# ersanjay16/Assignment--2-Group7-distributed-K-means

Measured on AMD Instinct MI355X. Metric: Lloyd iters/sec + points/sec, N=100M d=64 k=256, 1–8 GPUs; % of roofline, higher is better.
Workload: dtype f32; 1 GPU; c3: N=100000000 d=64 k=256; N=100000000, d=64, k=256, compute_sse=False, parallelism=dp1 (rows sharded, one RCCL all-reduce of k*(d+1) f64 per step)

## Files before the change

assignment--2-group7-distributed-k-means_amd/_lib.py:

```python
from __future__ import annotations

import ctypes
import os
import threading

HERE = os.path.dirname(os.path.abspath(__file__))
_KM_LIB = os.environ.get("KM_LIB")
LIB_PATH = os.path.join(HERE, "libkmeans_amd.so") if _KM_LIB in (None, "", "diag") else _KM_LIB
ROOT = os.path.dirname(HERE)
HEADER = os.path.join(ROOT, "include", "kmeans_amd.h")

KM_ABI_VERSION = 6
KM_OK = 0
KM_EMPTY = 1

KM_K_ASSIGN, KM_K_RESOLVE, KM_K_STATS, KM_K_UPDATE, KM_K_PREP, KM_K_SEED = range(6)
KERNEL_KINDS = {"assign": KM_K_ASSIGN, "resolve": KM_K_RESOLVE, "stats": KM_K_STATS, "update": KM_K_UPDATE,
                "prep": KM_K_PREP, "seed": KM_K_SEED}


KM_STOP_CONVERGED, KM_STOP_EMPTY, KM_STOP_NONFINITE = 1, 2, 3
KM_MAX_BATCH = 32


class KmStatus(ctypes.Structure):
    _fields_ = [("sse", ctypes.c_double), ("max_shift", ctypes.c_double), ("n_empty", ctypes.c_int32),
                ("nonfinite", ctypes.c_int32), ("q_rerank", ctypes.c_int32), ("q_full", ctypes.c_int32),
                ("ran", ctypes.c_int32), ("stop_reason", ctypes.c_int32), ("repaired", ctypes.c_int32),
                ("reserved", ctypes.c_int32)]


class KmInfo(ctypes.Structure):
    _fields_ = [("n", ctypes.c_int64), ("d", ctypes.c_int32), ("dp", ctypes.c_int32), ("k", ctypes.c_int32),
                ("kp", ctypes.c_int32), ("path", ctypes.c_int32), ("n_cu", ctypes.c_int32),
                ("device", ctypes.c_int32), ("fused_stats", ctypes.c_int32),
                ("delta_stats", ctypes.c_int32)]


_P = ctypes.c_void_p
_I32 = ctypes.c_int32
_I64 = ctypes.c_int64
_D = ctypes.c_double
_PD = ctypes.POINTER(ctypes.c_double)
_PI32 = ctypes.POINTER(ctypes.c_int32)
_PI64 = ctypes.POINTER(ctypes.c_int64)
_PF = ctypes.POINTER(ctypes.c_float)

SIGNATURES = {
    "km_abi_version": [],
    "km_device_count": [ctypes.POINTER(ctypes.c_int)],
    "km_create": [ctypes.c_int, ctypes.POINTER(_P)],
    "km_destroy": [_P],
    "km_set_stream": [_P, _P],
    "km_sync": [_P],
    "km_info_get": [_P, ctypes.POINTER(KmInfo)],
    "km_gated_rows": [_P, _PI64],
    "km_stats_route": [_P, _PI32, _PI32, _PI32, _PI32, _PI32],
    "km_load_begin": [_P, _I64, _I32],
    "km_load_rows": [_P, _I64, _PF, _I64],
    "km_generate_blobs": [_P, _I64, _I32, _I64, _I32, ctypes.c_float, ctypes.c_float, ctypes.c_uint64],
    "km_set_weights": [_P, _I64, _PD, _I64],
    "km_clear_weights": [_P],
    "km_sum_x": [_P, _PD],
    "km_set_sse": [_P, _I32],
    "km_set_screen": [_P, _I32],
    "km_get_screen": [_P, ctypes.POINTER(ctypes.c_int32)],
    "km_set_centroids": [_P, _PD, _I32, _I32],
    "km_get_centroids": [_P, _I32, _PD],
    "km_assign_stats": [_P],
    "km_stats_buffer": [_P, ctypes.POINTER(_P), _PI64],
    "km_bind_stats_buffer": [_P, _P],
    "km_update": [_P, ctypes.POINTER(KmStatus), _PI64],
    "km_batch_begin": [_P],
    "km_update_async": [_P, _D, _I64],
    "km_set_layout": [_P, _PI64, _I32, _I64, _I32],
    "km_repair_state": [_P, _PI32, _PI32],
    "km_repair_buffer": [_P, ctypes.POINTER(_P), _PI64],
    "km_bind_repair_buffer": [_P, _P],
    "km_repair_apply_async": [_P],
    "km_batch_end": [_P, ctypes.POINTER(KmStatus), _PI64, _PI32],
    "km_replace_rows": [_P, _PI32, _PD, _I32],
    "km_commit": [_P],
    "km_gather_rows": [_P, _PI64, _I32, _PD],
    "km_bernoulli_sample": [_P, ctypes.POINTER(ctypes.c_uint64), _PI64, _PI64, _I32, ctypes.c_double, _PI64,
                            ctypes.c_int64, _PI64],
    "km_seed_begin": [_P],
    "km_seed_update": [_P, _I32, _PD],
    "km_seed_sample": [_P, ctypes.c_uint64, _I32, _I64, _D, _D, _PI64, _I64, _PI64],
    "km_seed_weights": [_P, _I32, _PI64],
    "km_seed_read": [_P, _PD, _PI32],
    "km_seed_end": [_P],
    "km_predict": [_P, _PI32],
    "km_labels": [_P, _PI32],
    "km_profile": [_P, _I32],
    "km_profile_every": [_P, _I32],
    "km_prof_read": [_P, _I32, _PD, _PI64],
}

_lock = threading.Lock()
_lib = None


class KmError(RuntimeError):
    pass


def _pin_runtime():
    try:
        import torch
    except Exception:
        pass


def load(path: str = None):
    global _lib
    path = path or LIB_PATH
    with _lock:
        if _lib is not None:
            return _lib
        if not os.path.exists(path):
            raise KmError(f"HIP extension not built: {path} is missing "
                          f"(run `python -c 'import __graft_entry__ as g; g.build()'` or "
                          f"`make -C {os.path.join(HERE, 'csrc')}`)")
        _pin_runtime()
        lib = ctypes.CDLL(path, mode=ctypes.RTLD_GLOBAL)
        for name, args in SIGNATURES.items():
            fn = getattr(lib, name)
            fn.argtypes = args
            fn.restype = ctypes.c_int
        lib.km_last_error.argtypes = []
        lib.km_last_error.restype = ctypes.c_char_p
        _lib = lib
        return lib


def check(rc: int, what: str = "") -> int:
    if rc < 0:
        msg = load().km_last_error().decode(errors="replace")
        raise KmError(f"{what or 'kmeans_amd'} failed ({rc}): {msg}")
    return rc


def device_count() -> int:
    lib = load()
    n = ctypes.c_int(0)
    check(lib.km_device_count(ctypes.byref(n)), "km_device_count")
    return n.value


def exported_symbols():
    return list(SIGNATURES) + ["km_last_error"]
```

assignment--2-group7-distributed-k-means_amd/csrc/km_internal.h:

```cpp
#pragma once
#include <hip/hip_ext.h>
#include <hip/hip_runtime.h>
#include <stdint.h>

#include "../../include/kmeans_amd.h"

namespace km {

struct LaunchTiming {
  hipEvent_t start = nullptr, stop = nullptr;
};
extern thread_local LaunchTiming g_timing;
#define KM_TIMED_LAUNCH(KERNEL, GRID, BLOCK, LDS, STREAM, ...)                                               \
  do {                                                                                                     \
    if (::km::g_timing.start) {                                                                            \
      hipExtLaunchKernelGGL(KERNEL, GRID, BLOCK, LDS, STREAM, ::km::g_timing.start, ::km::g_timing.stop, 0, \
                            __VA_ARGS__);                                                                  \
      ::km::g_timing = ::km::LaunchTiming{};                                                               \
    } else {                                                                                               \
      hipLaunchKernelGGL(KERNEL, GRID, BLOCK, LDS, STREAM, __VA_ARGS__);                                    \
    }                                                                                                      \
  } while (0)

struct QEntry {
  uint32_t row;
  uint32_t i1;
  uint32_t i2;
  uint32_t kind;
};

struct DevStatus {
  double sse;
  double max_shift;
  int32_t n_empty;
  int32_t nonfinite;
  int32_t q_rerank;
  int32_t q_full;
  int32_t ran;
  int32_t stop;
  int32_t repaired;
  int32_t pad;
};
static_assert(sizeof(DevStatus) == 48, "layout of km_status");


struct QLayout {
  uint32_t seg;
  uint32_t nwaves;
};

struct Geometry {
  int64_t n;
  int32_t d;
  int32_t dp;
  int32_t k;
  int32_t kp;
};

hipError_t launch_prep_centroids(const double* C64, const Geometry& g, float* C32, double* cn2, float* cmax,
                                 float* cabs, double* C64T, double* C64P, const int* gate, hipStream_t s);
hipError_t launch_prep_small(const double* C64, const Geometry& g, float* C32, float* cmax, const int* gate,
                             hipStream_t s);
hipError_t launch_prep_split(const float* C32, const Geometry& g, const double* cn2, const float* xabs,
                             const float* cabs, _Float16* Chi, _Float16* Clo, float* cn2s, const int* gate, hipStream_t s);
hipError_t launch_absmax(const float* X, int64_t nfloats, float* out, hipStream_t s);
struct SmallTail {
  uint32_t* queue;
  uint32_t* qctr;
  uint32_t* done;
  int fold;
  const double* old;
  double* out;
  int64_t* counts;
  DevStatus* st;
  int* gate;
  double stop_tol;
  int dev_repair;
  float* C32n;
  float* cmaxn;
  int kp;
  uint32_t* qout = nullptr;
  int rev = 0;
};
hipError_t launch_assign_small(const float* X, const Geometry& g, const float* C32, const double* C64,
                               const float* cmax, int32_t* labels, double* stats, int fuse_stats, int want_sse,
                               int n_cu, const int* gate, hipStream_t s, const SmallTail& tail);
bool small_path_ok(const Geometry& g);
hipError_t launch_assign_mfma(const float* X, const Geometry& g, const _Float16* Chi, const _Float16* Clo,
                              const float* cn2s, const float* cmax, const float* xabs, const float* cabs,
                              int32_t* labels, QEntry* queue, uint32_t* qcount, int n_cu, QLayout* ql,
                              const int* gate, hipStream_t s, uint32_t* cand = nullptr, uint32_t* cand_ctr = nullptr,
                              uint32_t cand_cap = 0, int one = 0,
                              const float* C32 = nullptr, uint2* chg = nullptr, uint32_t* chg_cnt = nullptr);
int cand_rec_words();
size_t queue_capacity(int64_t n, int n_cu);
size_t qcount_words(int n_cu);
bool mfma_path_ok(const Geometry& g);
hipError_t launch_resolve(const float* X, const Geometry& g, const double* C64, const double* C64T,
                          const QEntry* queue, const uint32_t* qcount, const QLayout& ql, int32_t* labels,
                          double* stats, int n_cu, const int* gate, hipStream_t s, double* sse = nullptr,
                          const uint32_t* cand = nullptr, uint32_t cand_cap = 0, int delta = 0,
                          const float* sse_c32 = nullptr, uint2* chg = nullptr, const uint32_t* chg_cnt = nullptr,
                          const float* C32 = nullptr, const float* cmax = nullptr);
bool fused_path_ok(const Geometry& g);
#ifdef KM_DIAG
#endif
int diag_env(const char* name, int dflt);
enum { KM_SCREEN_X3 = 0, KM_SCREEN_X3_REFINE = 1, KM_SCREEN_FAST1 = 2, KM_SCREEN_FAST2 = 3 };
bool fast_path_ok(const Geometry& g);
hipError_t launch_fused(const float* X, const float* xnorm, const Geometry& g, const _Float16* Chi,
                        const _Float16* Clo, uint4* ChiF, uint4* CloF, const float* cn2s, const float* bnd,
                        const float* xabs, const float* cabs, int32_t* labels, QEntry* queue, uint32_t* qcount,
                        double* stats, int with_stats, int mode, int n_cu, QLayout* ql, const int* gate,
                        hipStream_t s, const float* C32, const float* cmax, float* bal, const double* C64P,
                        double* sse);
hipError_t launch_bound_consts(const float* cmax, const float* xabs, const float* cabs, const Geometry& g, float* bnd,
                               const int* gate, hipStream_t s);
bool fused16_ok(const Geometry& g);
hipError_t launch_row_norm(const float* X, const Geometry& g, float* xnorm, hipStream_t s);
bool stats_needs_sort(const Geometry& g, int extra);
void stats_ranges(const Geometry& g, int* fr_out, int* kr_out, int extra);
size_t sorted_stats_words(int64_t n, int k);
hipError_t launch_stats(const float* X, const Geometry& g, const int32_t* labels, const double* w, double* stats,
                        int n_cu, const int* gate, hipStream_t s, const double* C64, int c64s, const float* C32);
hipError_t launch_stats_sorted(const float* X, const Geometry& g, const int32_t* labels, const double* w,
                               double* stats, uint32_t* scratch, const double* C64P, int n_cu, const int* gate,
                               hipStream_t s);
bool update_one_ok(const Geometry& g);
hipError_t launch_update(double* stats, const double* C64_old, const Geometry& g, double* C64_new,
                         double* work, int64_t* counts, const uint32_t* qcount, uint32_t nq, DevStatus* status,
                         int* gate, double stop_tol, int dev_repair, hipStream_t s, int clear = 0,
                         float* C32 = nullptr, float* cmax = nullptr, int corr = 0, const double* wdiv = nullptr);
hipError_t launch_sum_x(const float* X, const Geometry& g, double* out, hipStream_t s);
hipError_t launch_scatter_rows(const int64_t* ids, const double* rows, int32_t n, int d, double* C, hipStream_t s);
hipError_t launch_gather_rows(const float* X, const Geometry& g, const int64_t* idx, int32_t n, double* out,
                              hipStream_t s);
hipError_t launch_repair(int* gate, const int64_t* counts, const Geometry& g, int64_t total, double neg_log_delta,
                         uint64_t seed, int32_t* empty, int32_t* pcounts, int64_t* picks, int64_t* samples, int cp,
                         const int64_t* sizes, const int64_t* bases, int nparts, const float* X, int64_t row0,
                         const double* C_old, double* C_new, DevStatus* st, double tol, hipStream_t s);
hipError_t launch_repair_pick(int* gate, const int64_t* counts, const Geometry& g, int64_t total,
                              double neg_log_delta, uint64_t seed, int32_t* empty, int32_t* pcounts, int64_t* picks,
                              int64_t* samples, int cp, const int64_t* sizes, const int64_t* bases, int nparts,
                              const float* X, int64_t row0, DevStatus* st, double* rows, int32_t* pending,
                              hipStream_t s);
hipError_t launch_repair_apply(int* gate, const Geometry& g, const int32_t* empty, const double* C_old,
                               double* C_new, DevStatus* st, double tol, const double* rows, const int32_t* pending,
                               hipStream_t s);
hipError_t launch_bernoulli(const uint64_t* seeds, const int64_t* sizes, const int64_t* bases, int nparts,
                            double fraction, int64_t* out, int cp, int32_t* counts, hipStream_t s);
bool s1_ok(const Geometry& g);
size_t s1_table_entries(const Geometry& g);
hipError_t launch_s1_color(const float* C32, const Geometry& g, int32_t* perm, const int* gate, hipStream_t s);
hipError_t launch_s1_prep(const double* C64, const float* C32, const Geometry& g, const int32_t* perm,
                          const float* cmax, const float* xabs, const float* cabs, float* cft, float* cn2o,
                          uint4* img, float* cst, const int* gate, hipStream_t s);
struct S1GateBufs;
hipError_t launch_s1(const float* X, const float* xnorm, const Geometry& g, const uint4* img, const float* cn2o,
                     const float* cft, const int32_t* perm, const float* cst, int32_t* labels,
                     QEntry* queue, uint32_t* qcount, uint2* chg, uint32_t* chg_cnt, int delta, int n_cu,
                     QLayout* ql, const int* gate, hipStream_t s, int rev = 0, double* sse = nullptr,
                     const S1GateBufs* gt = nullptr, int gdense = 0);
struct S1GateBufs {
  float* marg;
  uint2* wl;
  uint32_t* wl_cnt;
  double* cref;
  double* acc;
  float* accud;
};
bool s1_gate_ok(const Geometry& g);
hipError_t launch_s1_gate(const Geometry& g, const double* C64, const int32_t* labels, const S1GateBufs& b, int init,
                          const int32_t* init_dev, int n_cu, const int* gate, hipStream_t s);
size_t s1_chg_entries(const Geometry& g, int n_cu);
size_t s1_wave_slots(int n_cu);
bool s1_delta_ok(const Geometry& g, int n_cu);
hipError_t launch_s1_delta(const float* X, const Geometry& g, const uint2* chg, const uint32_t* chg_cnt,
                           double* stats, int n_cu, const int* gate, hipStream_t s, const uint32_t* qcount = nullptr);
hipError_t launch_chg_delta(const float* X, const Geometry& g, const uint2* chg, const uint32_t* chg_cnt, int nw,
                            uint32_t seg, double* stats, int n_cu, const int* gate, hipStream_t s,
                            const uint32_t* qcount = nullptr);
hipError_t launch_s1_apply(double* stats, double* full, int64_t len, int mode, const int* gate, hipStream_t s);
hipError_t launch_gen_blobs(float* X, const Geometry& g, int64_t row_offset, int32_t n_centers, float box,
                            float stddev, uint64_t seed, hipStream_t s);

__host__ __device__ inline uint64_t splitmix64(uint64_t z) {
  z += 0x9E3779B97F4A7C15ull;
  z = (z ^ (z >> 30)) * 0xBF58476D1CE4E5B9ull;
  z = (z ^ (z >> 27)) * 0x94D049BB133111EBull;
  return z ^ (z >> 31);
}

hipError_t launch_seed_init(double* D2, int32_t* near, int64_t n, hipStream_t s);
int seed_fold_blocks(int64_t n, int n_cu);
int seed_sample_blocks(int64_t n, int n_cu);
hipError_t launch_seed_fold(const float* X, const Geometry& g, const double* C64, const int32_t* labels,
                            int32_t first_id, double* D2, int32_t* near, double* part, int n_cu, hipStream_t s);
hipError_t launch_seed_sample(const double* D2, int64_t n, uint64_t seed, int32_t round, int64_t row0, double ell,
                              double phi, uint32_t* cnt, int64_t* offs, int64_t* out, int64_t cap, int n_cu,
                              hipStream_t s);
hipError_t launch_seed_weights(const int32_t* near, int64_t n, int32_t m_total, unsigned long long* counts, int n_cu,
                               hipStream_t s);

}
```

assignment--2-group7-distributed-k-means_amd/csrc/km_runtime.hip:

```cpp
#include <stdlib.h>
#include <string.h>

#include <algorithm>
#include <cmath>
#include <string>
#include <utility>
#include <vector>

#include "../../include/kmeans_amd.h"
#include "km_internal.h"

namespace {
thread_local std::string g_err;

int fail(int code, const std::string& msg) {
  g_err = msg;
  return code;
}

#define KM_HIP(call)                                                                               \
  do {                                                                                             \
    hipError_t e_ = (call);                                                                        \
    if (e_ != hipSuccess)                                                                          \
      return fail(KM_ERR_HIP, std::string(#call) + ": " + hipGetErrorString(e_) + " (" +           \
                                  std::to_string((int)e_) + ")");                                  \
  } while (0)

#define KM_REQUIRE(cond, code, msg) \
  do {                              \
    if (!(cond)) return fail(code, msg); \
  } while (0)

template <class T>
void dfree(T*& p) {
  if (p) (void)hipFree(p);
  p = nullptr;
}
template <class T>
void hfree(T*& p) {
  if (p) (void)hipHostFree(p);
  p = nullptr;
}

constexpr int kAllowedDp[] = {16, 32, 48, 64, 96, 128, 192, 256};

bool fused_disabled() { return km::diag_env("KM_FUSED", 1) == 0; }

size_t stats_len(const km::Geometry& g) { return (size_t)g.k * (g.d + 1) + 1; }
size_t stats_cap(const km::Geometry& g) { return stats_len(g) + (size_t)g.k; }

int choose_dp(int d) {
  for (int v : kAllowedDp)
    if (d <= v) return v;
  return (d + 15) / 16 * 16;
}
}

struct km_ctx {
  int device = 0;
  int n_cu = 256;
  hipStream_t own_stream = nullptr;
  hipStream_t stream = nullptr;
  km::Geometry g{};
  bool loaded = false;
  bool have_c = false;
  int path = 0;
  bool fused = false;
  int screen = km::KM_SCREEN_X3_REFINE;
  bool fast_blocked = false;
  int screen_forced = -1;
  bool s1 = false;
  bool mdelta_geo = false;
  uint2* chg_m = nullptr;
  uint32_t* chg_m_cnt = nullptr;
  bool s1_recolor = true;
  int s1_color_age = 0;
  int s1_batches = 0;
  int32_t* s1_perm = nullptr;
  float* s1_cft = nullptr;
  float* s1_cn2o = nullptr;
  uint4* s1_img = nullptr;
  float* s1_cst = nullptr;
  double* stats_full = nullptr;
  uint2* chg = nullptr;
  uint32_t* chg_cnt = nullptr;
  bool delta_ready = false;
  km::S1GateBufs gt{nullptr, nullptr, nullptr, nullptr, nullptr, nullptr};
  bool bounds_valid = false;
  bool last_gated = false;
  uint32_t gated_nw = 0;
  bool gated_dense = false;
  const int32_t* gate_init_dev = nullptr;
  bool x3_stale = true;
  bool sweep_rev = false;
  int stats_pending = 0;
  bool last_delta = false;
  bool sse_corr = false;
  float* bal = nullptr;
  bool stats_clean = false;
  bool rep_armed = false;
  float* X = nullptr;
  double* w = nullptr;
  int32_t* labels = nullptr;
  km::QEntry* queue = nullptr;
  uint32_t* qcount = nullptr;
  uint32_t* small_ctr = nullptr;
  bool assign_pending = false;
  bool stats_exported = false;
  uint32_t* cand = nullptr;
  uint32_t* cand_ctr = nullptr;
  uint32_t cand_cap = 0;
  km::QLayout ql{0, 0};
  double* moments = nullptr;
  bool want_sse = false;
  int64_t* idx_scratch = nullptr;
  double* rows_scratch = nullptr;
  int64_t scratch_rows = 0;
  int k_alloc = 0;
  double* C64_cur = nullptr;
  double* C64_new = nullptr;
  double* C64T = nullptr;
  double* C64P = nullptr;
  float* C32 = nullptr;
  _Float16* Chi = nullptr;
  _Float16* Clo = nullptr;
  double* cn2 = nullptr;
  float* cn2s = nullptr;
  float* cmax = nullptr;
  float* cabs = nullptr;
  float* xabs = nullptr;
  float* xnorm = nullptr;
  uint4* ChiF = nullptr;
  uint4* CloF = nullptr;
  float* bnd = nullptr;
  uint32_t* sort_scratch = nullptr;
  size_t sort_words = 0;
  double* stats_own = nullptr;
  double* stats = nullptr;
  double* work = nullptr;
  int64_t* counts_dev = nullptr;
  km::DevStatus* status_dev = nullptr;
  km::DevStatus* status_host = nullptr;
  int64_t* counts_host = nullptr;
  int* gate = nullptr;
  km::DevStatus* hist = nullptr;
  km::DevStatus* hist_host = nullptr;
  int64_t* hist_counts = nullptr;
  int64_t* hist_counts_host = nullptr;
  bool in_batch = false;
  int batch_n = 0;
  double* slot_cur[KM_MAX_BATCH] = {};
  double* slot_new[KM_MAX_BATCH] = {};
  bool rep_enabled = false;
  int rep_nparts = 0;
  int64_t rep_total = 0, rep_row0 = 0, rep_maxpart = 0;
  int64_t* rep_sizes = nullptr;
  int64_t* rep_bases = nullptr;
  int rep_cp = 0, rep_k = 0;
  int32_t* rep_empty = nullptr;
  int32_t* rep_pcounts = nullptr;
  int64_t* rep_picks = nullptr;
  int64_t* rep_samples = nullptr;
  int rep_mode = 0;
  double* rep_rows = nullptr;
  double* rep_rows_own = nullptr;
  int32_t* rep_pending = nullptr;
  bool rep_wait = false;
  double rep_tol = 0.0;
  bool rep_fold = false;
  bool seed_on = false;
  double* seed_d2 = nullptr;
  int32_t* seed_near = nullptr;
  double* seed_part = nullptr;
  uint32_t* seed_cnt = nullptr;
  int64_t* seed_offs = nullptr;
  int64_t* seed_out = nullptr;
  int64_t seed_out_cap = 0;
  float* pinned = nullptr;
  size_t pinned_floats = 0;
  hipEvent_t staged[2] = {nullptr, nullptr};
  int prof = 0;
  int prof_period = 1;
  int64_t prof_tick[KM_K_COUNT] = {};
  const double* prep_of = nullptr;
  struct Timed {
    hipEvent_t first, second;
    int64_t batch;
    int slot;
  };
  std::vector<Timed> ev[KM_K_COUNT];
  int64_t batch_seq = 0;
  std::vector<hipEvent_t> pool;

  hipEvent_t take_event() {
    if (!pool.empty()) {
      hipEvent_t e = pool.back();
      pool.pop_back();
      return e;
    }
    hipEvent_t e = nullptr;
    (void)hipEventCreate(&e);
    return e;
  }
};

namespace {

size_t stats_len(const km_ctx* c) { return c->w ? stats_cap(c->g) : stats_len(c->g); }

struct ProfScope {
  km_ctx* c;
  int kind;
  bool in_dispatch;
  hipEvent_t a = nullptr, b = nullptr;
  bool on;
  ProfScope(km_ctx* ctx, int k, bool dispatch = false)
      : c(ctx), kind(k), in_dispatch(dispatch),
        on(((c->prof >> k) & 1) && (c->prof_tick[k]++ % c->prof_period) == 0) {
    if (on) {
      a = c->take_event();
      b = c->take_event();
      if (in_dispatch)
        km::g_timing = km::LaunchTiming{a, b};
      else
        (void)hipEventRecord(a, c->stream);
    }
  }
  ~ProfScope() {
    if (on) {
      if (!in_dispatch) {
        (void)hipEventRecord(b, c->stream);
      } else if (km::g_timing.start) {
        km::g_timing = km::LaunchTiming{};
        (void)hipEventRecord(a, c->stream);
        (void)hipEventRecord(b, c->stream);
      }
      c->ev[kind].push_back({a, b, c->in_batch ? c->batch_seq : -1, c->batch_n});
    }
  }
};

void free_centroids(km_ctx* c) {
  dfree(c->C64_cur);
  dfree(c->C64_new);
  dfree(c->C64T);
  dfree(c->C64P);
  dfree(c->C32);
  dfree(c->Chi);
  dfree(c->Clo);
  dfree(c->cn2);
  dfree(c->cn2s);
  dfree(c->ChiF);
  dfree(c->CloF);
  dfree(c->bnd);
  c->bal = nullptr;
  dfree(c->cmax);
  dfree(c->cabs);
  dfree(c->stats_own);
  dfree(c->s1_perm);
  dfree(c->s1_cft);
  dfree(c->s1_cn2o);
  dfree(c->s1_img);
  dfree(c->s1_cst);
  dfree(c->stats_full);
  dfree(c->chg);
  dfree(c->chg_cnt);
  dfree(c->gt.marg);
  dfree(c->gt.wl);
  dfree(c->gt.wl_cnt);
  dfree(c->gt.cref);
  dfree(c->gt.acc);
  dfree(c->gt.accud);
  c->bounds_valid = false;
  c->last_gated = false;
  c->s1 = false;
  c->mdelta_geo = false;
  c->delta_ready = false;
  c->stats_pending = 0;
  dfree(c->work);
  dfree(c->counts_dev);
  dfree(c->status_dev);
  hfree(c->status_host);
  hfree(c->counts_host);
  dfree(c->hist);
  hfree(c->hist_host);
  dfree(c->hist_counts);
  hfree(c->hist_counts_host);
  c->in_batch = false;
  c->batch_n = 0;
  if (c->stats != nullptr && c->stats != c->stats_own) {
  }
  c->stats = nullptr;
  c->k_alloc = 0;
  c->have_c = false;
}

void free_seed(km_ctx* c) {
  dfree(c->seed_d2);
  dfree(c->seed_near);
  dfree(c->seed_part);
  dfree(c->seed_cnt);
  dfree(c->seed_offs);
  dfree(c->seed_out);
  c->seed_out_cap = 0;
  c->seed_on = false;
}

void free_data(km_ctx* c) {
  free_seed(c);
  dfree(c->X);
  dfree(c->w);
  dfree(c->labels);
  dfree(c->queue);
  dfree(c->qcount);
  dfree(c->small_ctr);
  c->assign_pending = false;
  dfree(c->cand);
  dfree(c->cand_ctr);
  c->cand_cap = 0;
  dfree(c->chg_m);
  dfree(c->chg_m_cnt);
  dfree(c->moments);
  dfree(c->xabs);
  dfree(c->xnorm);
  dfree(c->sort_scratch);
  c->sort_words = 0;
  dfree(c->idx_scratch);
  dfree(c->rows_scratch);
  c->scratch_rows = 0;
  c->loaded = false;
  c->delta_ready = false;
}

int ensure_x3(km_ctx* c) {
  if (!c->x3_stale) return KM_OK;
  KM_HIP(km::launch_prep_split(c->C32, c->g, c->cn2, c->xabs, c->cabs, c->Chi, c->Clo, c->cn2s, c->gate, c->stream));
  KM_HIP(km::launch_bound_consts(c->cmax, c->xabs, c->cabs, c->g, c->bnd, c->gate, c->stream));
  c->x3_stale = false;
  return KM_OK;
}

int prep(km_ctx* c, const double* src) {
  ProfScope ps(c, KM_K_PREP);
  c->prep_of = src;
  if (c->path == 1) {
    KM_HIP(km::launch_prep_small(src, c->g, c->C32, c->cmax, c->gate, c->stream));
    return KM_OK;
  }
  KM_HIP(km::launch_prep_centroids(src, c->g, c->C32, c->cn2, c->cmax, c->cabs, c->C64T, c->C64P, c->gate,
                                   c->stream));
  c->x3_stale = true;
  if (!c->s1) {
    const int rc = ensure_x3(c);
    if (rc != KM_OK) return rc;
  }
  if (c->s1) {
    if (c->s1_recolor) {
      KM_HIP(km::launch_s1_color(c->C32, c->g, c->s1_perm, c->gate, c->stream));
      c->s1_recolor = false;
    }
    KM_HIP(km::launch_s1_prep(src, c->C32, c->g, c->s1_perm, c->cmax, c->xabs, c->cabs, c->s1_cft, c->s1_cn2o,
                              c->s1_img, c->s1_cst, c->gate, c->stream));
  }
  return KM_OK;
}

int ensure_scratch(km_ctx* c, int64_t rows) {
  if (rows <= c->scratch_rows) return KM_OK;
  dfree(c->idx_scratch);
  dfree(c->rows_scratch);
  KM_HIP(hipMalloc(&c->idx_scratch, sizeof(int64_t) * rows));
  KM_HIP(hipMalloc(&c->rows_scratch, sizeof(double) * rows * std::max(1, c->g.d)));
  c->scratch_rows = rows;
  return KM_OK;
}

int prep(km_ctx* c) { return prep(c, c->C64_cur); }

void free_repair(km_ctx* c) {
  dfree(c->rep_empty);
  dfree(c->rep_pcounts);
  dfree(c->rep_picks);
  dfree(c->rep_samples);
  dfree(c->rep_rows_own);
  dfree(c->rep_pending);
  c->rep_rows = nullptr;
  c->rep_cp = 0;
  c->rep_k = 0;
}

void drop_layout(km_ctx* c) {
  free_repair(c);
  dfree(c->rep_sizes);
  dfree(c->rep_bases);
  c->rep_enabled = false;
  c->rep_armed = false;
  c->rep_wait = false;
  c->rep_mode = 0;
  c->rep_nparts = 0;
  c->rep_total = 0;
  c->rep_maxpart = 0;
  c->rep_row0 = 0;
}

double sample_fraction(int64_t num, int64_t total) {
  const double fraction = (double)num / (double)total;
  const double gamma = -std::log(0.00005) / (double)total;
  return std::min(1.0, fraction + gamma + std::sqrt(gamma * gamma + 2.0 * gamma * fraction));
}

int ensure_repair(km_ctx* c) {
  if (c->rep_k == c->g.k && c->rep_pcounts) return KM_OK;
  free_repair(c);
  const double f = sample_fraction(std::min<int64_t>(c->g.k, std::max<int64_t>(c->rep_total - 1, 1)),
                                   std::max<int64_t>(c->rep_total, 1));
  const double cpd = 4.0 * f * (double)c->rep_maxpart + 64.0;
  KM_REQUIRE(cpd < (double)(1 << 26), KM_ERR_ARG, "km_update_async: repair buffers too large");
  c->rep_cp = (int)cpd;
  const size_t slots = (size_t)c->rep_cp * c->rep_nparts;
  KM_HIP(hipMalloc(&c->rep_empty, sizeof(int32_t) * c->g.k));
  KM_HIP(hipMalloc(&c->rep_pcounts, sizeof(int32_t) * c->rep_nparts));
  KM_HIP(hipMemsetAsync(c->rep_pcounts, 0, sizeof(int32_t) * c->rep_nparts, c->stream));
  KM_HIP(hipMalloc(&c->rep_picks, sizeof(int64_t) * slots));
  KM_HIP(hipMalloc(&c->rep_samples, sizeof(int64_t) * slots));
  KM_HIP(hipMalloc(&c->rep_pending, sizeof(int32_t)));
  KM_HIP(hipMemsetAsync(c->rep_pending, 0, sizeof(int32_t), c->stream));
  if (c->rep_mode == 2) {
    KM_HIP(hipMalloc(&c->rep_rows_own, sizeof(double) * (size_t)c->g.k * std::max(1, c->g.d)));
    c->rep_rows = c->rep_rows_own;
  }
  c->rep_k = c->g.k;
  return KM_OK;
}

bool next_sweep(km_ctx* c) {
  if ((double)c->g.n * c->g.dp * 4.0 > 8.0 * (1ull << 30)) return false;
  c->sweep_rev = !c->sweep_rev;
  return c->sweep_rev;
}

km::SmallTail small_tail(km_ctx* c) {
  km::SmallTail t{};
  t.queue = reinterpret_cast<uint32_t*>(c->queue);
  t.qctr = c->small_ctr;
  t.done = c->small_ctr + 1;
  t.kp = c->g.kp;
  t.qout = c->qcount;
  t.rev = next_sweep(c);
  return t;
}

bool fold_ok(km_ctx* c) {
  return c->in_batch && c->path == 1 && km::update_one_ok(c->g) && c->stats == c->stats_own && !c->stats_exported &&
         !(c->rep_enabled && c->rep_armed) && !c->w;
}

int run_assign(km_ctx* c, bool with_stats);

#ifndef KM_PAIR_RESCORE
#define KM_PAIR_RESCORE 1
#endif

bool one_screen(km_ctx* c) {
  if (c->path != 2 || c->fused || c->g.dp % 32 != 0 || c->g.dp > 256) return false;
  if (c->screen_forced == KM_SCREEN_ONE) return true;
  return c->screen_forced < 0 && !c->s1;
}

bool use_s1(km_ctx* c, bool with_stats) {
  if (!c->s1) return false;
  if (c->screen_forced >= 0 && c->screen_forced != KM_SCREEN_S1) return false;
  return !with_stats || (c->delta_ready && !c->stats_exported && km::s1_delta_ok(c->g, c->n_cu));
}

int stats_route(const km_ctx* c) {
  if (c->w) return km::stats_needs_sort(c->g, 2) ? 2 : 1;
  if (c->path == 1 || c->fused) return 0;
  return km::stats_needs_sort(c->g, 1) ? 2 : 1;
}

int run_stats(km_ctx* c, bool sse) {
  const km::Geometry& g = c->g;
  ProfScope ps(c, KM_K_STATS);
  if (stats_route(c) == 2) {
    const size_t words = km::sorted_stats_words(g.n, g.k);
    if (words > c->sort_words) {
      dfree(c->sort_scratch);
      KM_HIP(hipMalloc(&c->sort_scratch, sizeof(uint32_t) * words));
      c->sort_words = words;
    }
    KM_REQUIRE(!c->w || c->path == 2, KM_ERR_UNSUPPORTED,
               "km_assign_stats: weighted statistics need the MFMA path at this k");
    KM_HIP(km::launch_stats_sorted(c->X, g, c->labels, c->w, c->stats, c->sort_scratch, sse ? c->C64P : nullptr,
                                   c->n_cu, c->gate, c->stream));
  } else {
    const bool small = c->path == 1;
    KM_HIP(km::launch_stats(c->X, g, c->labels, c->w, c->stats, c->n_cu, c->gate, c->stream,
                            sse ? (small ? c->C64_cur : c->C64P) : nullptr, small ? g.d : g.dp,
                            sse ? c->C32 : nullptr));
  }
  return KM_OK;
}

int apply_stats(km_ctx* c, const double** upd_src = nullptr, bool clear = false) {
  const int kind = c->stats_pending;
  c->stats_pending = 0;
  if (upd_src) *upd_src = c->stats;
  if (!c->s1 && !c->mdelta_geo) return KM_OK;
  const bool keep = kind == 2 || kind == 1;
  const bool zero = kind == 2 && clear && upd_src;
  if (keep)
    KM_HIP(km::launch_s1_apply(c->stats, c->stats_full, (int64_t)stats_len(c), kind == 2 ? (zero ? 2 : 1) : 0,
                               c->gate, c->stream));
  if (zero) {
    *upd_src = c->stats_full;
    c->stats_clean = true;
  }
  c->delta_ready = keep;
  return KM_OK;
}

int take_sse_corr(km_ctx* c) {
  const bool v = c->sse_corr;
  c->sse_corr = false;
  return v ? 1 : 0;
}

int flush_assign(km_ctx* c) {
  if (!c->assign_pending) return KM_OK;
  c->assign_pending = false;
  return run_assign(c, true);
}

int run_assign(km_ctx* c, bool with_stats) {
  const km::Geometry& g = c->g;
  if (c->prep_of != c->C64_cur) {
    const int rc = prep(c);
    if (rc != KM_OK) return rc;
  }
  c->ql = km::QLayout{0, 0};
  if (with_stats && c->stats_pending == 2) {
    c->delta_ready = false;
  }
  const bool sse = with_stats && c->want_sse;
  double* sse_slot = c->stats + (size_t)g.k * (g.d + 1);
  const bool bounds_were_valid = c->bounds_valid;
  c->bounds_valid = false;
  if (!use_s1(c, with_stats)) c->gate_init_dev = nullptr;
  if (with_stats) c->last_gated = false;
  if (with_stats && !c->stats_clean) KM_HIP(hipMemsetAsync(c->stats, 0, sizeof(double) * stats_len(c), c->stream));
  if (with_stats) c->stats_clean = false;
  if (c->path == 1) {
    ProfScope ps(c, KM_K_ASSIGN, true);
    KM_HIP(km::launch_assign_small(c->X, g, c->C32, c->C64_cur, c->cmax, c->labels, c->stats, with_stats ? 1 : 0,
                                   sse ? 1 : 0, c->n_cu, c->gate, c->stream, small_tail(c)));
    c->ql = km::QLayout{0, g.n > 0 ? 1u : 0u};
    return KM_OK;
  }
  if (with_stats) {
    c->stats_pending = 1;
    c->last_delta = false;
    c->sse_corr = false;
  }
  if (use_s1(c, with_stats)) {
    double* s1_sse = sse ? sse_slot : nullptr;
    const bool gated = with_stats && !s1_sse && c->fused && g.n > 0 && km::s1_gate_ok(g);
    bool gdense = false;
    if (gated) {
      if (!c->gt.marg) {
        KM_HIP(hipMalloc(&c->gt.marg, sizeof(float) * (size_t)g.n));
        KM_HIP(hipMalloc(&c->gt.wl, sizeof(uint2) * km::s1_chg_entries(g, c->n_cu)));
        KM_HIP(hipMalloc(&c->gt.wl_cnt, sizeof(uint32_t) * km::s1_wave_slots(c->n_cu)));
        KM_HIP(hipMalloc(&c->gt.cref, sizeof(double) * (size_t)g.k * g.d));
        KM_HIP(hipMemsetAsync(c->gt.cref, 0, sizeof(double) * (size_t)g.k * g.d, c->stream));
        KM_HIP(hipMalloc(&c->gt.acc, sizeof(double) * (size_t)g.k));
        KM_HIP(hipMalloc(&c->gt.accud, sizeof(float) * 2 * (size_t)g.k));
        KM_HIP(hipMemsetAsync(c->gt.acc, 0, sizeof(double) * (size_t)g.k, c->stream));
        KM_HIP(hipMemsetAsync(c->gt.accud, 0, sizeof(float) * 2 * (size_t)g.k, c->stream));
      }
      gdense = !bounds_were_valid;
      ProfScope ps(c, KM_K_PREP);
      KM_HIP(km::launch_s1_gate(g, c->C64_cur, c->labels, c->gt, gdense ? 2 : 0, c->gate_init_dev, c->n_cu, c->gate,
                                c->stream));
    }
    c->gate_init_dev = nullptr;
    {
      ProfScope ps(c, KM_K_ASSIGN, true);
      KM_HIP(km::launch_s1(c->X, c->xnorm, g, c->s1_img, c->s1_cn2o, c->s1_cft, c->s1_perm, c->s1_cst,
                           c->labels, c->queue, c->qcount, c->chg, c->chg_cnt, with_stats ? 1 : 0, c->n_cu,
                           &c->ql, c->gate, c->stream, gated ? 0 : next_sweep(c), s1_sse,
                           gated ? &c->gt : nullptr, gdense ? 1 : 0));
    }
    if (gated) {
      c->bounds_valid = true;
      c->last_gated = true;
      c->gated_nw = c->ql.nwaves;
      c->gated_dense = gdense;
    }
    {
      ProfScope ps(c, KM_K_RESOLVE);
      KM_HIP(km::launch_resolve(c->X, g, c->C64_cur, c->C64T, c->queue, c->qcount, c->ql, c->labels, nullptr,
                                c->n_cu, c->gate, c->stream, s1_sse, nullptr, 0, with_stats ? 1 : 0,
                                s1_sse ? c->C32 : nullptr, c->chg, c->chg_cnt, c->C32, c->cmax));
    }
    if (with_stats) {
      ProfScope ps(c, KM_K_STATS);
      KM_HIP(km::launch_s1_delta(c->X, g, c->chg, c->chg_cnt, c->stats, c->n_cu, c->gate, c->stream, c->qcount));
    }
    if (with_stats) {
      c->stats_pending = 2;
      c->last_delta = true;
      c->sse_corr = s1_sse != nullptr;
    }
    return KM_OK;
  }
  if (c->fused) {
    {
      const int rc = ensure_x3(c);
      if (rc != KM_OK) return rc;
    }
    {
      ProfScope ps(c, KM_K_ASSIGN, true);
      KM_HIP(km::launch_fused(c->X, c->xnorm, g, c->Chi, c->Clo, c->ChiF, c->CloF, c->cn2s, c->bnd, c->xabs, c->cabs,
                              c->labels, c->queue, c->qcount, c->stats, with_stats ? 1 : 0,
                              (with_stats || c->screen >= km::KM_SCREEN_FAST1) ? c->screen : km::KM_SCREEN_X3_REFINE,
                              c->n_cu, &c->ql, c->gate, c->stream, c->C32, c->cmax, c->bal, c->C64P,
                              sse ? sse_slot : nullptr));
    }
    {
      ProfScope ps(c, KM_K_RESOLVE);
      KM_HIP(km::launch_resolve(c->X, g, c->C64_cur, c->C64T, c->queue, c->qcount, c->ql, c->labels,
                                with_stats ? c->stats : nullptr, c->n_cu, c->gate, c->stream,
                                sse ? sse_slot : nullptr, nullptr, 0, 0, nullptr, nullptr, nullptr, c->C32, c->cmax));
    }
    return KM_OK;
  }
  if (c->s1 && !c->fused && (c->screen_forced < 0 || c->screen_forced == KM_SCREEN_S1)) {
    {
      ProfScope ps(c, KM_K_ASSIGN, true);
      KM_HIP(km::launch_s1(c->X, c->xnorm, g, c->s1_img, c->s1_cn2o, c->s1_cft, c->s1_perm, c->s1_cst, c->labels,
                           c->queue, c->qcount, c->chg, c->chg_cnt, 0, c->n_cu, &c->ql, c->gate, c->stream,
                           next_sweep(c)));
    }
    {
      ProfScope ps(c, KM_K_RESOLVE);
      KM_HIP(km::launch_resolve(c->X, g, c->C64_cur, c->C64T, c->queue, c->qcount, c->ql, c->labels, nullptr,
                                c->n_cu, c->gate, c->stream, nullptr, nullptr, 0, 0, nullptr, nullptr, nullptr, c->C32,
                                c->cmax));
    }
  } else {
  if (!c->cand && g.dp <= 256) {
    const int64_t cap = std::min<int64_t>(std::max<int64_t>(g.n, 1024), (int64_t)1 << 22);
    KM_HIP(hipMalloc(&c->cand, sizeof(uint32_t) * km::cand_rec_words() * (size_t)cap));
    KM_HIP(hipMalloc(&c->cand_ctr, sizeof(uint32_t)));
    c->cand_cap = (uint32_t)cap;
  }
  {
    const int rc = ensure_x3(c);
    if (rc != KM_OK) return rc;
  }
  const bool mdelta = with_stats && c->mdelta_geo && c->delta_ready && !c->want_sse && !c->stats_exported;
  if (mdelta && !c->chg_m) {
    KM_HIP(hipMalloc(&c->chg_m, sizeof(uint2) * km::queue_capacity(std::max<int64_t>(g.n, 1), c->n_cu)));
    KM_HIP(hipMalloc(&c->chg_m_cnt, sizeof(uint32_t) * km::qcount_words(c->n_cu)));
  }
  {
    ProfScope ps(c, KM_K_ASSIGN);
    KM_HIP(km::launch_assign_mfma(c->X, g, c->Chi, c->Clo, c->cn2s, c->cmax, c->xabs, c->cabs, c->labels, c->queue,
                                  c->qcount, c->n_cu, &c->ql, c->gate, c->stream, c->cand, c->cand_ctr,
                                  c->cand_cap, one_screen(c) ? 1 : 0, KM_PAIR_RESCORE ? c->C32 : nullptr,
                                  mdelta ? c->chg_m : nullptr, mdelta ? c->chg_m_cnt : nullptr));
  }
  {
    ProfScope ps(c, KM_K_RESOLVE);
    KM_HIP(km::launch_resolve(c->X, g, c->C64_cur, c->C64T, c->queue, c->qcount, c->ql, c->labels, nullptr, c->n_cu,
                              c->gate, c->stream, nullptr, c->cand, c->cand_cap, mdelta ? 1 : 0, nullptr,
                              mdelta ? c->chg_m : nullptr, mdelta ? c->chg_m_cnt : nullptr, c->C32, c->cmax));
  }
  if (mdelta) {
    ProfScope ps(c, KM_K_STATS);
    KM_HIP(km::launch_chg_delta(c->X, g, c->chg_m, c->chg_m_cnt, (int)c->ql.nwaves, c->ql.seg, c->stats, c->n_cu,
                                c->gate, c->stream, c->qcount));
    c->stats_pending = 2;
    c->last_delta = true;
    return KM_OK;
  }
  }
  if (with_stats) return run_stats(c, sse);
  return KM_OK;
}

int run_assign_weighted(km_ctx* c) {
  int rc = run_assign(c, false);
  if (rc != KM_OK) return rc;
  c->delta_ready = false;
  c->stats_pending = 0;
  c->last_delta = false;
  c->last_gated = false;
  c->sse_corr = false;
  c->gate_init_dev = nullptr;
  KM_HIP(hipMemsetAsync(c->stats, 0, sizeof(double) * stats_len(c), c->stream));
  c->stats_clean = false;
  return run_stats(c, c->want_sse);
}

const double* wdiv_of(const km_ctx* c, const double* src) { return c->w ? src + stats_len(c->g) : nullptr; }

}

extern "C" {

int km_abi_version(void) { return KM_ABI_VERSION; }

const char* km_last_error(void) { return g_err.c_str(); }

int km_device_count(int* out) {
  KM_REQUIRE(out, KM_ERR_ARG, "km_device_count: null out");
  int n = 0;
  hipError_t e = hipGetDeviceCount(&n);
  if (e != hipSuccess) n = 0;
  *out = n;
  return KM_OK;
}

int km_create(int device, km_ctx** out) {
  KM_REQUIRE(out, KM_ERR_ARG, "km_create: null out");
  *out = nullptr;
  int n = 0;
  KM_HIP(hipGetDeviceCount(&n));
  KM_REQUIRE(device >= 0 && device < n, KM_ERR_ARG,
             "km_create: device " + std::to_string(device) + " out of range (" + std::to_string(n) + " devices)");
  KM_HIP(hipSetDevice(device));
  hipDeviceProp_t prop;
  KM_HIP(hipGetDeviceProperties(&prop, device));
  KM_REQUIRE(std::string(prop.gcnArchName).rfind("gfx950", 0) == 0, KM_ERR_UNSUPPORTED,
             std::string("km_create: kernels are built for gfx950 (MI355X), device is ") + prop.gcnArchName);
  km_ctx* c = new km_ctx();
  c->device = device;
  c->n_cu = prop.multiProcessorCount;
  hipError_t e = hipStreamCreateWithFlags(&c->own_stream, hipStreamNonBlocking);
  if (e != hipSuccess) {
    delete c;
    return fail(KM_ERR_HIP, std::string("hipStreamCreate: ") + hipGetErrorString(e));
  }
  c->stream = c->own_stream;
  e = hipMalloc(&c->gate, sizeof(int));
  if (e == hipSuccess) e = hipMemset(c->gate, 0, sizeof(int));
  if (e != hipSuccess) {
    (void)hipStreamDestroy(c->own_stream);
    delete c;
    return fail(KM_ERR_HIP, std::string("km_create: ") + hipGetErrorString(e));
  }
  *out = c;
  return KM_OK;
}

int km_destroy(km_ctx* c) {
  if (!c) return KM_OK;
  (void)hipSetDevice(c->device);
  (void)hipStreamSynchronize(c->stream);
  free_centroids(c);
  free_data(c);
  hfree(c->pinned);
  for (auto& e : c->staged)
    if (e) (void)hipEventDestroy(e);
  for (auto& v : c->ev)
    for (auto& p : v) {
      (void)hipEventDestroy(p.first);
      (void)hipEventDestroy(p.second);
    }
  for (auto e : c->pool) (void)hipEventDestroy(e);
  dfree(c->gate);
  free_repair(c);
  dfree(c->rep_sizes);
  dfree(c->rep_bases);
  if (c->own_stream) (void)hipStreamDestroy(c->own_stream);
  delete c;
  return KM_OK;
}

int km_set_stream(km_ctx* c, void* s) {
  KM_REQUIRE(c, KM_ERR_ARG, "null ctx");
  KM_HIP(hipSetDevice(c->device));
  {
    const int rcf = flush_assign(c);
    if (rcf != KM_OK) return rcf;
  }
  KM_HIP(hipStreamSynchronize(c->stream));
  c->stream = s ? reinterpret_cast<hipStream_t>(s) : c->own_stream;
  return KM_OK;
}

int km_sync(km_ctx* c) {
  KM_REQUIRE(c, KM_ERR_ARG, "null ctx");
  KM_HIP(hipSetDevice(c->device));
  {
    const int rcf = flush_assign(c);
    if (rcf != KM_OK) return rcf;
  }
  KM_HIP(hipStreamSynchronize(c->stream));
  return KM_OK;
}

int km_info_get(km_ctx* c, km_info* out) {
  KM_REQUIRE(c && out, KM_ERR_ARG, "null arg");
  out->n = c->g.n;
  out->d = c->g.d;
  out->dp = c->g.dp;
  out->k = c->g.k;
  out->kp = c->g.kp;
  out->path = c->path;
  out->n_cu = c->n_cu;
  out->device = c->device;
  out->fused_stats = (c->path == 1) || c->fused;
  out->delta_stats = c->last_delta ? 1 : 0;
  return KM_OK;
}

int km_gated_rows(km_ctx* c, int64_t* out) {
  KM_REQUIRE(c && out, KM_ERR_ARG, "null arg");
  *out = -1;
  if (!c->last_gated || !c->gt.wl_cnt || c->gated_nw == 0) return KM_OK;
  if (c->gated_dense) {
    *out = c->g.n;
    return KM_OK;
  }
  KM_HIP(hipSetDevice(c->device));
  std::vector<uint32_t> cnt(c->gated_nw);
  KM_HIP(hipMemcpyAsync(cnt.data(), c->gt.wl_cnt, sizeof(uint32_t) * cnt.size(), hipMemcpyDeviceToHost, c->stream));
  KM_HIP(hipStreamSynchronize(c->stream));
  int64_t total = 0;
  for (uint32_t v : cnt) total += v;
  *out = total;
  return KM_OK;
}

int km_stats_route(km_ctx* c, int32_t* route, int32_t* cluster_ranges, int32_t* kr, int32_t* feature_ranges,
                   int32_t* fr) {
  KM_REQUIRE(c && route && cluster_ranges && kr && feature_ranges && fr, KM_ERR_ARG, "km_stats_route: null arg");
  KM_REQUIRE(c->have_c && c->path != 0, KM_ERR_STATE, "km_stats_route: set centroids of a supported geometry first");
  *route = stats_route(c);
  *cluster_ranges = *kr = *feature_ranges = *fr = 0;
  if (*route == 0) return KM_OK;
  int f = 0, r = 0;
  km::stats_ranges(c->g, &f, &r, c->w ? 2 : 1);
  KM_REQUIRE(f > 0 && r > 0, KM_ERR_UNSUPPORTED, "km_stats_route: no table split for this geometry");
  *fr = f;
  *kr = r;
  *feature_ranges = c->g.dp / f;
  *cluster_ranges = (c->g.k + r - 1) / r;
  return KM_OK;
}

int km_load_begin(km_ctx* c, int64_t n, int32_t d) {
  KM_REQUIRE(c, KM_ERR_ARG, "null ctx");
  KM_REQUIRE(n >= 0 && n < (int64_t)UINT32_MAX, KM_ERR_ARG, "km_load_begin: n out of range");
  KM_REQUIRE(d > 0, KM_ERR_ARG, "km_load_begin: d must be positive");
  KM_HIP(hipSetDevice(c->device));
  {
    const int rcf = flush_assign(c);
    if (rcf != KM_OK) return rcf;
  }
  KM_HIP(hipStreamSynchronize(c->stream));
  free_data(c);
  free_centroids(c);
  drop_layout(c);
  c->g = km::Geometry{};
  c->g.n = n;
  c->g.d = d;
  c->g.dp = choose_dp(d);
  const int64_t rows = std::max<int64_t>(n, 1);
  KM_HIP(hipMalloc(&c->X, sizeof(float) * rows * c->g.dp));
  KM_HIP(hipMemsetAsync(c->X, 0, sizeof(float) * rows * c->g.dp, c->stream));
  KM_HIP(hipMalloc(&c->labels, sizeof(int32_t) * rows));
  KM_HIP(hipMalloc(&c->queue, sizeof(km::QEntry) * km::queue_capacity(rows, c->n_cu)));
  KM_HIP(hipMalloc(&c->qcount, sizeof(uint32_t) * km::qcount_words(c->n_cu)));
  KM_HIP(hipMalloc(&c->small_ctr, sizeof(uint32_t) * 3));
  KM_HIP(hipMemsetAsync(c->small_ctr, 0, sizeof(uint32_t) * 3, c->stream));
  KM_HIP(hipMalloc(&c->moments, sizeof(double) * (d + 1)));
  KM_HIP(hipMalloc(&c->xabs, sizeof(float)));
  KM_HIP(hipMalloc(&c->xnorm, sizeof(float) * rows));
  KM_HIP(hipMemsetAsync(c->xabs, 0, sizeof(float), c->stream));
  KM_HIP(hipStreamSynchronize(c->stream));
  c->loaded = true;
  return KM_OK;
}

int km_load_rows(km_ctx* c, int64_t row0, const float* rows, int64_t nrows) {
  KM_REQUIRE(c && c->loaded, KM_ERR_STATE, "km_load_rows: call km_load_begin first");
  KM_REQUIRE(row0 >= 0 && nrows >= 0 && row0 + nrows <= c->g.n, KM_ERR_ARG, "km_load_rows: rows out of range");
  if (nrows == 0) return KM_OK;
  KM_REQUIRE(rows, KM_ERR_ARG, "km_load_rows: null rows");
  KM_HIP(hipSetDevice(c->device));
  {
    const int rcf = flush_assign(c);
    if (rcf != KM_OK) return rcf;
  }
  c->delta_ready = false;
  c->bounds_valid = false;
  const int d = c->g.d, dp = c->g.dp;
  const size_t chunk_floats = (size_t)16 << 20;
  if (!c->pinned) {
    KM_HIP(hipHostMalloc(&c->pinned, 2 * chunk_floats * sizeof(float), hipHostMallocDefault));
    c->pinned_floats = chunk_floats;
    for (auto& e : c->staged) KM_HIP(hipEventCreateWithFlags(&e, hipEventDisableTiming));
  }
  const int64_t per = std::max<int64_t>(1, (int64_t)(c->pinned_floats / d));
  KM_REQUIRE((size_t)d <= c->pinned_floats, KM_ERR_ARG, "km_load_rows: row wider than the staging buffer");
  int half = 0;
  bool used[2] = {false, false};
  for (int64_t r = 0; r < nrows; r += per, half ^= 1) {
    const int64_t m = std::min(per, nrows - r);
    float* buf = c->pinned + (size_t)half * c->pinned_floats;
    if (used[half]) KM_HIP(hipEventSynchronize(c->staged[half]));
    memcpy(buf, rows + r * d, sizeof(float) * m * d);
    KM_HIP(hipMemcpy2DAsync(c->X + (row0 + r) * dp, sizeof(float) * dp, buf, sizeof(float) * d,
                            sizeof(float) * d, m, hipMemcpyHostToDevice, c->stream));
    KM_HIP(hipEventRecord(c->staged[half], c->stream));
    used[half] = true;
    KM_HIP(km::launch_absmax(c->X + (row0 + r) * dp, m * dp, c->xabs, c->stream));
    km::Geometry sub = c->g;
    sub.n = m;
    KM_HIP(km::launch_row_norm(c->X + (row0 + r) * dp, sub, c->xnorm + row0 + r, c->stream));
  }
  KM_HIP(hipStreamSynchronize(c->stream));
  return KM_OK;
}

static int weights_mode_changed(km_ctx* c) {
  c->delta_ready = false;
  c->bounds_valid = false;
  c->last_gated = false;
  c->last_delta = false;
  c->stats_pending = 0;
  c->sse_corr = false;
  c->stats_clean = false;
  c->stats = c->stats_own;
  return KM_OK;
}

int km_set_weights(km_ctx* c, int64_t row0, const double* w, int64_t nrows) {
  KM_REQUIRE(c && c->loaded, KM_ERR_STATE, "km_set_weights: call km_load_begin first");
  KM_REQUIRE(!c->in_batch, KM_ERR_STATE, "km_set_weights: inside a batch");
  KM_REQUIRE(row0 >= 0 && nrows >= 0 && row0 + nrows <= c->g.n, KM_ERR_ARG, "km_set_weights: rows out of range");
  KM_REQUIRE(nrows == 0 || w, KM_ERR_ARG, "km_set_weights: null weights");
  KM_HIP(hipSetDevice(c->device));
  {
    const int rcf = flush_assign(c);
    if (rcf != KM_OK) return rcf;
  }
  KM_HIP(hipStreamSynchronize(c->stream));
  if (!c->w) {
    const int64_t rows = std::max<int64_t>(c->g.n, 1);
    std::vector<double> ones((size_t)std::min<int64_t>(rows, (int64_t)1 << 20), 1.0);
    KM_HIP(hipMalloc(&c->w, sizeof(double) * rows));
    for (int64_t r = 0; r < rows; r += (int64_t)ones.size())
      KM_HIP(hipMemcpy(c->w + r, ones.data(), sizeof(double) * std::min<int64_t>((int64_t)ones.size(), rows - r),
                       hipMemcpyHostToDevice));
    weights_mode_changed(c);
  }
  const int64_t per = (int64_t)8 << 20;
  for (int64_t r = 0; r < nrows; r += per) {
    const int64_t m = std::min(per, nrows - r);
    KM_HIP(hipMemcpyAsync(c->w + row0 + r, w + r, sizeof(double) * m, hipMemcpyHostToDevice, c->stream));
    KM_HIP(hipStreamSynchronize(c->stream));
  }
  c->delta_ready = false;
  return KM_OK;
}

int km_clear_weights(km_ctx* c) {
  KM_REQUIRE(c, KM_ERR_ARG, "null ctx");
  KM_REQUIRE(!c->in_batch, KM_ERR_STATE, "km_clear_weights: inside a batch");
  if (!c->w) return KM_OK;
  KM_HIP(hipSetDevice(c->device));
  KM_HIP(hipStreamSynchronize(c->stream));
  dfree(c->w);
  return weights_mode_changed(c);
}

int km_generate_blobs(km_ctx* c, int64_t n, int32_t d, int64_t global_row0, int32_t n_centers, float box,
                      float stddev, uint64_t seed) {
  KM_REQUIRE(c, KM_ERR_ARG, "null ctx");
  KM_REQUIRE(n_centers > 0, KM_ERR_ARG, "n_centers must be positive");
  int rc = km_load_begin(c, n, d);
  if (rc != KM_OK) return rc;
  KM_HIP(km::launch_gen_blobs(c->X, c->g, global_row0, n_centers, box, stddev, seed, c->stream));
  KM_HIP(km::launch_absmax(c->X, c->g.n * c->g.dp, c->xabs, c->stream));
  KM_HIP(km::launch_row_norm(c->X, c->g, c->xnorm, c->stream));
  KM_HIP(hipStreamSynchronize(c->stream));
  return KM_OK;
}

int km_sum_x(km_ctx* c, double* out) {
  KM_REQUIRE(c && c->loaded && out, KM_ERR_STATE, "km_sum_x: no data");
  KM_HIP(hipSetDevice(c->device));
  KM_HIP(hipMemsetAsync(c->moments, 0, sizeof(double) * (c->g.d + 1), c->stream));
  KM_HIP(km::launch_sum_x(c->X, c->g, c->moments, c->stream));
  KM_HIP(hipMemcpyAsync(out, c->moments, sizeof(double) * c->g.d, hipMemcpyDeviceToHost, c->stream));
  KM_HIP(hipStreamSynchronize(c->stream));
  return KM_OK;
}

int km_set_screen(km_ctx* c, int32_t mode) {
  KM_REQUIRE(c, KM_ERR_ARG, "null ctx");
  KM_REQUIRE(mode >= -1 && mode <= KM_SCREEN_ONE, KM_ERR_ARG, "km_set_screen: mode must be -1..5");
#ifndef KM_DIAG
  KM_REQUIRE(mode <= km::KM_SCREEN_X3_REFINE || mode == KM_SCREEN_S1 || mode == KM_SCREEN_ONE, KM_ERR_UNSUPPORTED,
             "km_set_screen: fast screens (modes 2, 3) are in the diagnostic build only");
#endif
  c->screen_forced = mode;
  if (mode >= 0 && mode != KM_SCREEN_S1 && mode != KM_SCREEN_ONE) c->screen = mode;
  return KM_OK;
}

int km_get_screen(km_ctx* c, int32_t* mode) {
  KM_REQUIRE(c && mode, KM_ERR_ARG, "null ctx");
  *mode = (use_s1(c, true) || (c->s1 && !c->fused && (c->screen_forced < 0 || c->screen_forced == KM_SCREEN_S1)))
              ? KM_SCREEN_S1
              : one_screen(c) ? KM_SCREEN_ONE : c->screen;
  return KM_OK;
}

int km_set_sse(km_ctx* c, int32_t enable) {
  KM_REQUIRE(c, KM_ERR_ARG, "null ctx");
  {
    const int rcf = flush_assign(c);
    if (rcf != KM_OK) return rcf;
  }
  c->want_sse = enable != 0;
  return KM_OK;
}

int km_set_centroids(km_ctx* c, const double* C, int32_t k, int32_t d) {
  KM_REQUIRE(c && c->loaded, KM_ERR_STATE, "km_set_centroids: load data first");
  KM_REQUIRE(C, KM_ERR_ARG, "km_set_centroids: null C");
  KM_REQUIRE(k > 0, KM_ERR_ARG, "km_set_centroids: k must be positive");
  KM_REQUIRE(d == c->g.d, KM_ERR_ARG,
             "km_set_centroids: d=" + std::to_string(d) + " != data d=" + std::to_string(c->g.d));
  KM_HIP(hipSetDevice(c->device));
  {
    const int rcf = flush_assign(c);
    if (rcf != KM_OK) return rcf;
  }
  if (k != c->k_alloc) {
    KM_HIP(hipStreamSynchronize(c->stream));
    double* external = (c->stats && c->stats != c->stats_own) ? c->stats : nullptr;
    (void)external;
    free_centroids(c);
    c->g.k = k;
    c->g.kp = (k + 63) / 64 * 64;
    const int kp = c->g.kp, dp = c->g.dp;
    KM_HIP(hipMalloc(&c->C64_cur, sizeof(double) * k * d));
    KM_HIP(hipMalloc(&c->C64_new, sizeof(double) * k * d));
    KM_HIP(hipMalloc(&c->C64T, sizeof(double) * k * d));
    KM_HIP(hipMalloc(&c->C64P, sizeof(double) * kp * dp));
    KM_HIP(hipMalloc(&c->C32, sizeof(float) * kp * dp));
    KM_HIP(hipMalloc(&c->Chi, sizeof(_Float16) * kp * dp));
    KM_HIP(hipMalloc(&c->Clo, sizeof(_Float16) * kp * dp));
    KM_HIP(hipMalloc(&c->cn2, sizeof(double) * kp));
    KM_HIP(hipMalloc(&c->cn2s, sizeof(float) * kp));
    KM_HIP(hipMalloc(&c->ChiF, sizeof(_Float16) * kp * dp));
    KM_HIP(hipMalloc(&c->CloF, sizeof(_Float16) * kp * dp));
    KM_HIP(hipMalloc(&c->bnd, sizeof(float) * 16));
    c->bal = c->bnd + 4;
    KM_HIP(hipMalloc(&c->cmax, sizeof(float)));
    KM_HIP(hipMalloc(&c->cabs, sizeof(float)));
    KM_HIP(hipMalloc(&c->stats_own, sizeof(double) * stats_cap(c->g)));
    KM_HIP(hipMalloc(&c->work, sizeof(double) * 3 * k));
    KM_HIP(hipMalloc(&c->counts_dev, sizeof(int64_t) * k));
    KM_HIP(hipMalloc(&c->status_dev, sizeof(km::DevStatus)));
    KM_HIP(hipHostMalloc(&c->status_host, sizeof(km::DevStatus), hipHostMallocDefault));
    KM_HIP(hipHostMalloc(&c->counts_host, sizeof(int64_t) * k, hipHostMallocDefault));
    KM_HIP(hipMalloc(&c->hist, sizeof(km::DevStatus) * KM_MAX_BATCH));
    KM_HIP(hipHostMalloc(&c->hist_host, sizeof(km::DevStatus) * KM_MAX_BATCH, hipHostMallocDefault));
    KM_HIP(hipMalloc(&c->hist_counts, sizeof(int64_t) * (size_t)k * KM_MAX_BATCH));
    KM_HIP(hipHostMalloc(&c->hist_counts_host, sizeof(int64_t) * (size_t)k * KM_MAX_BATCH, hipHostMallocDefault));
    c->stats = c->stats_own;
    c->stats_clean = false;
    c->k_alloc = k;
    if (km::small_path_ok(c->g))
      c->path = 1;
    else if (km::mfma_path_ok(c->g))
      c->path = 2;
    else
      c->path = 0;
    c->fused = (c->path == 2) && km::fused_path_ok(c->g) && !fused_disabled();
    c->s1 = (c->path == 2) && (!c->fused || km::fused16_ok(c->g)) && km::s1_ok(c->g) &&
            km::diag_env("KM_S1", 1) != 0;
    c->mdelta_geo = (c->path == 2) && !c->fused && !c->s1 && c->g.dp % 32 == 0 && c->g.dp <= 128 &&
                    c->g.k <= 65535 && km::diag_env("KM_MDELTA", 1) != 0;
    if (c->mdelta_geo) KM_HIP(hipMalloc(&c->stats_full, sizeof(double) * stats_cap(c->g)));
    if (c->s1) {
      const size_t nt = km::s1_table_entries(c->g);
      KM_HIP(hipMalloc(&c->s1_perm, sizeof(int32_t) * nt));
      KM_HIP(hipMalloc(&c->s1_cft, sizeof(float) * nt * (dp + 4)));
      KM_HIP(hipMalloc(&c->s1_cn2o, sizeof(float) * kp));
      KM_HIP(hipMalloc(&c->s1_img, sizeof(_Float16) * kp * dp));
      KM_HIP(hipMalloc(&c->s1_cst, sizeof(float) * 8));
      KM_HIP(hipMalloc(&c->stats_full, sizeof(double) * stats_cap(c->g)));
      KM_HIP(hipMalloc(&c->chg, sizeof(uint2) * km::s1_chg_entries(c->g, c->n_cu)));
      KM_HIP(hipMalloc(&c->chg_cnt, sizeof(uint32_t) * km::s1_wave_slots(c->n_cu)));
    }
  }
  c->s1_recolor = true;
  c->s1_color_age = 0;
  c->s1_batches = 0;
  c->delta_ready = false;
  c->bounds_valid = false;
  c->stats_pending = 0;
  KM_HIP(hipMemcpyAsync(c->C64_cur, C, sizeof(double) * k * d, hipMemcpyHostToDevice, c->stream));
  int rc = prep(c);
  if (rc != KM_OK) return rc;
  KM_HIP(hipStreamSynchronize(c->stream));
  c->have_c = true;
  c->screen = c->screen_forced >= 0 ? c->screen_forced : km::KM_SCREEN_X3_REFINE;
  c->fast_blocked = false;
  c->rep_armed = c->rep_enabled;
  return KM_OK;
}

int km_get_centroids(km_ctx* c, int32_t which, double* out) {
  KM_REQUIRE(c && c->have_c && out, KM_ERR_STATE, "km_get_centroids: no centroids");
  KM_HIP(hipSetDevice(c->device));
  {
    const int rcf = flush_assign(c);
    if (rcf != KM_OK) return rcf;
  }
  const double* src = which ? c->C64_new : c->C64_cur;
  KM_HIP(hipMemcpyAsync(out, src, sizeof(double) * c->g.k * c->g.d, hipMemcpyDeviceToHost, c->stream));
  KM_HIP(hipStreamSynchronize(c->stream));
  return KM_OK;
// ... 651 lines not shown
```

assignment--2-group7-distributed-k-means_amd/csrc/km_s1_gate.h:

```cpp
#pragma once
#include <math.h>
#include <stdint.h>

#if defined(__HIPCC__) || defined(__CUDACC__)
#define KM_S1G_FN __host__ __device__ inline
#else
#define KM_S1G_FN inline
#endif

namespace km {

constexpr float S1G_U = 5.9604644775390625e-08f;
constexpr float S1G_TINY = 1e-30f;

KM_S1G_FN float s1g_up(float v) { return fmaf(fabsf(v), 8.0f * S1G_U, v) + S1G_TINY; }
KM_S1G_FN float s1g_dn(float v) { return fmaf(fabsf(v), -8.0f * S1G_U, v) - S1G_TINY; }

KM_S1G_FN float s1g_sqrt(float v) {
#if defined(__HIP_DEVICE_COMPILE__)
  return __builtin_amdgcn_sqrtf(v);
#else
  return sqrtf(v);
#endif
}

KM_S1G_FN float s1g_shift(double sq) {
  const double v = sqrt(sq) * (1.0 + 1e-12);
  const float f = (float)v;
  const float r = fmaf(f, 0x1p-23f, f) + S1G_TINY;
  return (r <= 3.0e38f) ? r : INFINITY;
}

KM_S1G_FN float s1g_step(float marg, float sl, float so) { return s1g_dn(marg - s1g_up(sl + so)); }

struct S1GRow {
  float is2;
  float E;
  float xlo;
  float xhi;
};

KM_S1G_FN S1GRow s1g_row(float s, float E_scaled, float xs) {
  S1GRow r;
  r.is2 = 1.0f / (s * s);
  r.E = s1g_up(E_scaled * r.is2);
  r.xhi = s1g_up(xs * (1.0f + 64.0f * S1G_U));
  r.xlo = s1g_dn(xs * (1.0f - 64.0f * S1G_U));
  return r;
}

KM_S1G_FN bool s1g_scale_ok(float s) { return s >= 0x1p-30f && s <= 0x1p30f; }

KM_S1G_FN float s1g_ub(float key, float rp, const S1GRow& r) {
  const float p = key * r.is2;
  float v = s1g_up(p + s1g_up(rp * fabsf(p)));
  v = s1g_up(v + r.E);
  v = s1g_up(v + r.xhi);
  v = !(v < 0x1p-96f) ? v : 0x1p-96f;
  return s1g_up(s1g_up(s1g_sqrt(v)));
}

KM_S1G_FN float s1g_lb(float key, float rp, const S1GRow& r) {
  const float p = key * r.is2;
  float v = s1g_dn(p - s1g_up(rp * fabsf(p)));
  v = s1g_dn(v - r.E);
  v = s1g_dn(v + r.xlo);
  return (v >= 0x1p-96f) ? s1g_dn(s1g_dn(s1g_sqrt(v))) : 0.0f;
}

KM_S1G_FN float s1g_margin(float lb, float ub) {
  const float m = s1g_dn(lb - ub);
  return (fabsf(m) <= 3.0e38f) ? m : 0.0f;
}

KM_S1G_FN double s1g_acc_add(double acc, float sl, float so) {
  return (acc + ((double)sl + (double)so)) * (1.0 + 0x1p-50);
}
KM_S1G_FN float s1g_acc_up(double acc) {
  const float f = (float)acc;
  const float r = fmaf(f, 0x1p-23f, f) + S1G_TINY;
  return (r <= 3.0e38f) ? r : INFINITY;
}
KM_S1G_FN float s1g_acc_dn(double acc) {
  if (!(acc <= 3.0e38)) return 0.0f;
  const float f = (float)acc;
  const float r = fmaf(f, -0x1p-23f, f) - S1G_TINY;
  return r > 0.0f ? r : 0.0f;
}
KM_S1G_FN double s1g_acc_pass(double acc, float sl, float so, float top, bool reset, float* up, float* dn) {
  const bool wild = !(top <= 3.0e38f);
  const double a = (reset || wild) ? 0.0 : s1g_acc_add(acc, sl, so);
  *up = (wild && !reset) ? INFINITY : s1g_acc_up(a);
  *dn = s1g_acc_dn(a);
  return a;
}
KM_S1G_FN float s1g_base(float marg, float acc_dn) {
  const float b = s1g_dn(marg + acc_dn);
  return (fabsf(b) <= 3.0e38f) ? b : 0.0f;
}
KM_S1G_FN bool s1g_keep(float base, float acc_up) { return base > acc_up; }

KM_S1G_FN float s1g_xnorm(float xs) {
  float v = s1g_up(xs * (1.0f + 64.0f * S1G_U));
  v = !(v < 0x1p-96f) ? v : 0x1p-96f;
  return s1g_up(s1g_up(s1g_sqrt(v)));
}

}
```

assignment--2-group7-distributed-k-means_amd/csrc/km_screen1.hip:

```cpp
#include <float.h>

#include <type_traits>

#include "km_internal.h"
#include "km_s1_gate.h"
#include "km_s1_ring.h"

namespace km {

namespace {

typedef _Float16 f16x8 __attribute__((ext_vector_type(8)));
typedef float f32x4 __attribute__((ext_vector_type(4)));
typedef float f32x2 __attribute__((ext_vector_type(2)));
typedef _Float16 f16x2 __attribute__((ext_vector_type(2)));

constexpr float U24 = 5.9604644775390625e-08f;
constexpr float U16 = 4.8828125e-04f;
#ifndef KM_S1_LMAX
#define KM_S1_LMAX 8
#endif
constexpr int S1_LMAX = KM_S1_LMAX;
#ifndef KM_S1_NBUF
#define KM_S1_NBUF 0
#endif
#ifndef KM_S1_ABL
#define KM_S1_ABL 0
#endif
constexpr int ceil_log2_c(int v) { return v <= 1 ? 0 : 1 + ceil_log2_c((v + 1) / 2); }
#ifndef KM_S1_W12
#define KM_S1_W12 1
#endif
#ifndef KM_S1_W12_C4
#define KM_S1_W12_C4 1
#endif
constexpr int s1_waves(int ns2, int nb) {
  return ((KM_S1_W12 && ns2 == 2 && nb == 8) || (KM_S1_W12_C4 && ns2 == 1 && nb == 32)) ? 12 : 8;
}

constexpr int S1_MAX_WAVES = 12;
constexpr int s1_ring(int ns2, int nb) { return s1_waves(ns2, nb) == 12 ? 12 : 16; }

constexpr bool s1_batched(int ns2) { return ns2 <= 2; }
#ifndef KM_S1_SERP
#define KM_S1_SERP 1
#endif
#ifndef KM_S1_TT
#define KM_S1_TT 1
#endif
constexpr int s1_tiles(int ns2) { return ns2 == 1 ? KM_S1_TT : 1; }

constexpr size_t s1_lds_bytes(int ns2, int nb, bool table) {
  const int dp = 32 * ns2, kp = 32 * nb, nt = 32 << ceil_log2_c(nb);
  return (size_t)kp * dp * 2 + (table ? (size_t)nt * (dp + 4) * 4 : 0) + (size_t)kp * 4 + (size_t)nt * 4 +
         (s1_batched(ns2) ? (size_t)s1_waves(ns2, nb) * s1_ring(ns2, nb) * (dp * 4 + 16 + 128) : 0);
}
constexpr bool s1_table_global(int ns2, int nb) { return s1_lds_bytes(ns2, nb, true) > 160 * 1024; }
#ifndef KM_S1_GATE
#define KM_S1_GATE 1
#endif
constexpr size_t s1_gate_ring_lds(int ns2, int nb) { return (size_t)s1_waves(ns2, nb) * s1_ring(ns2, nb) * 4; }
constexpr size_t s1_gate_lds(int ns2, int nb) { return s1_gate_ring_lds(ns2, nb) + (size_t)32 * nb * 4; }
constexpr bool s1_gated_with(int ns2, int nb, size_t extra) {
  return KM_S1_GATE && s1_batched(ns2) && s1_tiles(ns2) == 1 && !s1_table_global(ns2, nb) &&
         s1_lds_bytes(ns2, nb, true) + extra <= 160 * 1024;
}
constexpr bool s1_gated(int ns2, int nb) { return s1_gated_with(ns2, nb, s1_gate_lds(ns2, nb)); }
constexpr bool s1_gated_kept(int ns2, int nb) {
  return s1_gated(ns2, nb) == s1_gated_with(ns2, nb, s1_gate_ring_lds(ns2, nb));
}
static_assert(s1_gated_kept(2, 2) && s1_gated_kept(2, 4) && s1_gated_kept(2, 6) && s1_gated_kept(2, 8) &&
                  s1_gated_kept(1, 2) && s1_gated_kept(1, 4) && s1_gated_kept(1, 6) && s1_gated_kept(1, 8) &&
                  s1_gated_kept(1, 12) && s1_gated_kept(1, 16),
              "the lower totals' LDS table must not cost a geometry its gate");
static_assert(!KM_S1_GATE || !KM_S1_W12 || s1_gated(2, 8), "the c3 geometry is gated");


__device__ __forceinline__ uint32_t f2u(float v) { return __float_as_uint(v); }
__device__ __forceinline__ float u2f(uint32_t v) { return __uint_as_float(v); }

__device__ __forceinline__ float min_raw(float a, float b) {
  float r;
  asm("v_min_f32 %0, %1, %2" : "=v"(r) : "v"(a), "v"(b));
  return r;
}
__device__ __forceinline__ float min3_raw(float a, float b, float c) {
  float r;
  asm("v_min3_f32 %0, %1, %2, %3" : "=v"(r) : "v"(a), "v"(b), "v"(c));
  return r;
}

__device__ __forceinline__ float quad_min(float v) {
  auto p = __builtin_amdgcn_permlane16_swap(f2u(v), f2u(v), false, false);
  v = min_raw(u2f(p[0]), u2f(p[1]));
  p = __builtin_amdgcn_permlane32_swap(f2u(v), f2u(v), false, false);
  return min_raw(u2f(p[0]), u2f(p[1]));
}
__device__ __forceinline__ float quad_sum(float v) {
  auto p = __builtin_amdgcn_permlane16_swap(f2u(v), f2u(v), false, false);
  v = u2f(p[0]) + u2f(p[1]);
  p = __builtin_amdgcn_permlane32_swap(f2u(v), f2u(v), false, false);
  return u2f(p[0]) + u2f(p[1]);
}
__device__ __forceinline__ int32_t quad_min_i(int32_t v) {
  auto p = __builtin_amdgcn_permlane16_swap((uint32_t)v, (uint32_t)v, false, false);
  v = min((int32_t)p[0], (int32_t)p[1]);
  p = __builtin_amdgcn_permlane32_swap((uint32_t)v, (uint32_t)v, false, false);
  return min((int32_t)p[0], (int32_t)p[1]);
}
__device__ __forceinline__ int32_t mono(uint32_t b) { return (int32_t)(b ^ ((uint32_t)((int32_t)b >> 31) >> 1)); }
__device__ __forceinline__ uint32_t unmono(int32_t v) { return (uint32_t)v ^ ((uint32_t)(v >> 31) >> 1); }
__device__ __forceinline__ uint32_t quad_add_u(uint32_t v) {
  auto p = __builtin_amdgcn_permlane16_swap(v, v, false, false);
  v = p[0] + p[1];
  p = __builtin_amdgcn_permlane32_swap(v, v, false, false);
  return p[0] + p[1];
}

__device__ __forceinline__ float s1_scale(float xabs, float cabs) {
  const float m = fmaxf(xabs, cabs);
  if (!(m > 0.0f) || !(m < 3.0e38f)) return 1.0f;
  int e;
  (void)frexpf(m, &e);
  return ldexpf(1.0f, 14 - e);
}

}

struct S1Geo {
  int nb, mb, ns2;
};

template <int DPC, int NTH>
__global__ __launch_bounds__(NTH) void k_s1_color(const float* __restrict__ C32, int k, int dp, int nb, int mb,
                                                  int32_t* __restrict__ perm, const int* __restrict__ gate) {
  if (*gate) return;
  __shared__ unsigned int cmin[32];
  __shared__ int cnt[32];
  __shared__ int cls[NTH];
  const int t = threadIdx.x;
  float cv[DPC];
#pragma unroll
  for (int f = 0; f < DPC; ++f) cv[f] = (t < k && f < dp) ? C32[(size_t)t * dp + f] : 0.0f;
  if (t < 32) cnt[t] = 0;
  cls[t] = -1;
  __syncthreads();
  for (int j = 0; j < k; ++j) {
    if (t < 32) cmin[t] = 0x7F800000u;
    __syncthreads();
    if (t < j) {
      float s = 0.0f;
#pragma unroll
      for (int f = 0; f < DPC; ++f) {
        const float df = cv[f] - C32[(size_t)j * dp + f];
        s = fmaf(df, df, s);
      }
      atomicMin(&cmin[cls[t]], __float_as_uint(s));
    }
    __syncthreads();
    if (t < 64) {
      uint64_t key = 0;
      if (t < 32 && cnt[t] < nb) key = ((uint64_t)(cmin[t] + 1u) << 8) | (uint64_t)(31 - t);
#pragma unroll
      for (int o = 32; o >= 1; o >>= 1) {
        const uint64_t other = __shfl_xor(key, o);
        key = other > key ? other : key;
      }
      if (t == 0) {
        const int c = 31 - (int)(key & 255u);
        const int m = cnt[c];
        cls[j] = c;
        cnt[c] = m + 1;
        perm[(c << mb) | m] = j;
      }
    }
    __syncthreads();
  }
  for (int i = t; i < (32 << mb); i += blockDim.x) {
    const int c = i >> mb, m = i & ((1 << mb) - 1);
    if (m >= cnt[c]) perm[i] = -1;
  }
}

__global__ __launch_bounds__(64) void k_s1_prep(const double* __restrict__ C64, const float* __restrict__ C32, int k,
                                                int d, int dp, S1Geo sg, const int32_t* __restrict__ perm,
                                                const float* __restrict__ cmax, const float* __restrict__ xabs,
                                                const float* __restrict__ cabs, float* __restrict__ cft,
                                                float* __restrict__ cn2o, uint4* __restrict__ img,
                                                float* __restrict__ cst,
                                                const int* __restrict__ gate) {
  if (*gate) return;
  const int b = blockIdx.x, th = threadIdx.x;
  const int nt = 32 << sg.mb;
  const float s = s1_scale(*xabs, *cabs);
  const int cs = dp + 4;
  if (b < nt) {
    const int chain = b >> sg.mb, member = b & ((1 << sg.mb) - 1);
    const int j = member < sg.nb ? perm[b] : -1;
    for (int f = th; f < cs; f += 64) cft[(size_t)b * cs + f] = (j >= 0 && f < d) ? C32[(size_t)j * dp + f] : 0.0f;
    if (member >= sg.nb) return;
    const int cb = chain >> 4, M = chain & 15;
    if (th == 0) {
      double nn = 0.0;
      if (j >= 0)
        for (int f = 0; f < d; ++f) nn = fma(C64[(size_t)j * d + f], C64[(size_t)j * d + f], nn);
      cn2o[32 * member + 16 * cb + M] = j >= 0 ? (float)(nn * (double)s * (double)s) : 1e30f;
    }
    const int fq = dp / 4;
    if (th < 4 * sg.ns2) {
      const int q = th / sg.ns2, t = th - q * sg.ns2;
      f16x8 v;
#pragma unroll
      for (int e = 0; e < 8; ++e) {
        const int f = fq * q + 8 * t + e;
        v[e] = (j >= 0 && f < d) ? (_Float16)(-2.0f * s * C32[(size_t)j * dp + f]) : (_Float16)0.0f;
      }
      img[((size_t)(member * 2 + cb) * sg.ns2 + t) * 64 + 16 * q + M] = __builtin_bit_cast(uint4, v);
    }
    return;
  }
  if (th == 0) {
    const float cm = *cmax * s, ca = *cabs * (1.0f + U24) * s, xa = *xabs * s;
    const float sq = sqrtf((float)dp) * 1.0001f, nm = (float)sg.ns2;
    const float e1 = 1.25f * (2.0f * s * cm * (2.0f * U16 + U16 * U16 + 2.0f * U24) +
                              nm * 4.0f * U24 * 2.0f * s * cm * (1.0f + 2.0f * U16) +
                              ldexpf(1.0f, -25) * s * sq * (1.0f + U16));
    const float e0 = 1.25f * (U24 * cm * cm + nm * (4.0f * U24 * cm * cm +
                                                     28.0f * U24 * 2.0f * ca * xa * (1.0f + U16) * (1.0f + U16)) +
                              ldexpf(1.0f, -24) * sq * cm);
    cst[0] = s;
    cst[1] = e1 * 1.0001f;
    cst[2] = e0 * 1.0001f + 1e-30f;
    cst[3] = U24 * *cmax * 1.01f + 1e-37f;
  }
}

struct S1Args {
  const float* X;
  const float* xnorm;
  int64_t n;
  int k, d;
  uint32_t seg;
  const uint4* img;
  const float* cn2o;
  const float* cft;
  const int32_t* perm;
  const float* cst;
  int32_t* labels;
  QEntry* queue;
  uint32_t* qcount;
  uint2* chg;
  uint32_t* chg_cnt;
  double* sse;
  const int* gate;
  const uint2* wl;
  const uint32_t* wl_cnt;
  float* marg;
  const float* acc_dn;
};

template <int NS2, int NB, int MODE, bool REV = false, bool SSE = false, int GATED = 0>
__global__ __launch_bounds__(s1_waves(NS2, NB) * 64, s1_waves(NS2, NB) / 4) void k_s1(S1Args A) {
  if (*A.gate) return;
  constexpr int S1_WAVES = s1_waves(NS2, NB);
  constexpr int S1_RING = s1_ring(NS2, NB);
  static_assert(S1_RING == 12 || S1_RING == 16, "ring sizes covered by s1_ring_check");
  static_assert(16 <= 2 * S1_RING && S1_TILE_ROWS == 16, "a tile may complete at most two batches");
  static_assert(!GATED || (MODE == 1 && !REV && !SSE && s1_batched(NS2)), "the gated instance: delta mode, batched");
  constexpr bool LIST = GATED == 1;
  constexpr bool MARG = GATED != 0;
  constexpr int DP = 32 * NS2;
  constexpr int FQ = 8 * NS2;
  constexpr int KP = 32 * NB;
  constexpr int MB = ceil_log2_c(NB);
  constexpr int NT = 32 << MB;
  constexpr int CS = DP + 4;
  constexpr uint32_t SLOTM = (uint32_t)NT - 1u;
  constexpr uint32_t KMASK = ~SLOTM;
  constexpr float RHO = (float)SLOTM * 1.1920928955078125e-07f * 1.0001f;
  constexpr bool BATCH = s1_batched(NS2);
  constexpr bool TG = s1_table_global(NS2, NB);
  extern __shared__ __attribute__((aligned(16))) char smem[];
  const uint4* sImg = reinterpret_cast<const uint4*>(smem);
  float* sCf = reinterpret_cast<float*>(smem + KP * DP * 2);
  float* sCn = sCf + (TG ? 0 : NT * CS);
  int32_t* sPerm = reinterpret_cast<int32_t*>(sCn + KP);
  float* sRx = reinterpret_cast<float*>(sPerm + NT);
  uint4* sRm = reinterpret_cast<uint4*>(sRx + S1_WAVES * S1_RING * DP);
  float4* sRh = reinterpret_cast<float4*>(sRm + S1_WAVES * S1_RING);
  float* sRl = reinterpret_cast<float*>(sRh + S1_WAVES * S1_RING * 8);
  float* sAd = sRl + S1_WAVES * S1_RING;

  const int lane = threadIdx.x & 63;
  const int wave = threadIdx.x >> 6;
  const int c16 = lane & 15;
  const int q = lane >> 4;
  {
    uint4* di = reinterpret_cast<uint4*>(smem);
    for (int i = threadIdx.x; i < KP * DP / 8; i += S1_WAVES * 64) di[i] = A.img[i];
    if constexpr (!TG) {
      const float4* src = reinterpret_cast<const float4*>(A.cft);
      float4* dst = reinterpret_cast<float4*>(sCf);
      for (int i = threadIdx.x; i < NT * CS / 4; i += S1_WAVES * 64) dst[i] = src[i];
    }
    for (int i = threadIdx.x; i < KP; i += S1_WAVES * 64) sCn[i] = A.cn2o[i];
    for (int i = threadIdx.x; i < NT; i += S1_WAVES * 64) sPerm[i] = A.perm[i];
    if constexpr (MARG)
      for (int i = threadIdx.x; i < KP; i += S1_WAVES * 64) sAd[i] = i < A.k ? A.acc_dn[i] : 0.0f;
  }
  __syncthreads();

  const float s = A.cst[0], e1 = A.cst[1], e0 = A.cst[2], gam = A.cst[3];
  const uint32_t n = (uint32_t)A.n;
  const uint32_t ntiles = (n + 15u) / 16u;
  const uint32_t gw = blockIdx.x * S1_WAVES + wave;
  const uint32_t nw = gridDim.x * S1_WAVES;
  QEntry* wq = A.queue + (size_t)gw * A.seg;
  uint2* wc = A.chg + (size_t)gw * A.seg;
  uint32_t qn = 0, qf = 0, cc = 0;
  double ssa = 0.0;
  auto resid = [&](bool act, uint32_t slot, const float4* xv) {
    if constexpr (SSE) {
      const uint32_t sl = act ? slot : 0u;
      const float4* cp = TG ? reinterpret_cast<const float4*>(A.cft + sl * CS + FQ * q)
                            : reinterpret_cast<const float4*>(sCf + sl * CS + FQ * q);
      double r = 0.0;
#pragma unroll
      for (int u = 0; u < FQ / 4; ++u) {
        const float4 c = cp[u];
        const float4 x = xv[u];
        const double e0 = (double)x.x - (double)c.x, e1 = (double)x.y - (double)c.y;
        const double e2 = (double)x.z - (double)c.z, e3 = (double)x.w - (double)c.w;
        r = fma(e0, e0, r);
        r = fma(e1, e1, r);
        r = fma(e2, e2, r);
        r = fma(e3, e3, r);
      }
      ssa += act ? r : 0.0;
    } else {
      (void)act;
      (void)slot;
      (void)xv;
    }
  };
  const uint32_t qbits = (uint32_t)(4 * q) << MB;

  struct BufDense {
    float4 x[FQ / 4];
    float xn;
    int32_t old;
  };
  struct BufList {
    float4 x[FQ / 4];
  };
  using Buf = typename std::conditional<LIST, BufList, BufDense>::type;
  const uint2* wlp = nullptr;
  uint32_t wln = 0;
  uint2 wg0 = make_uint2(0xFFFFFFFFu, 0u), wg1 = wg0, wg2 = wg0;
  uint32_t wsub = 0;
  const bool gscale = MARG && s1g_scale_ok(s);
  auto wfetch = [&](uint32_t g) { return wlp[min(g * 64u + (uint32_t)lane, A.seg - 1u)]; };
  auto wmark = [&](uint32_t g, uint2 v) {
    return make_uint2(g * 64u + (uint32_t)lane < wln ? v.x : 0xFFFFFFFFu, v.y);
  };
  auto wpick = [&](uint32_t v, uint32_t sub) {
    return (uint32_t)__builtin_amdgcn_ds_bpermute((int)((sub * 16u + (uint32_t)c16) * 4u), (int)v);
  };
  if constexpr (LIST) {
    const uint32_t gwu = (uint32_t)__builtin_amdgcn_readfirstlane((int)gw);
    wlp = A.wl + (size_t)gwu * A.seg;
    wln = (uint32_t)__builtin_amdgcn_readfirstlane((int)min(A.wl_cnt[gwu], A.seg));
    wg0 = wmark(0u, wfetch(0u));
    wg1 = wmark(1u, wfetch(1u));
  }
  auto tmap = [&](uint32_t t) { return (REV && t < ntiles) ? ntiles - 1u - t : t; };
  auto load = [&](uint32_t tile, Buf& B) {
    uint32_t row;
    if constexpr (LIST) {
      row = tile < 4u ? wpick(wg0.x, tile) : wpick(wg1.x, 0u);
    } else {
      row = tmap(tile) * 16u + (uint32_t)c16;
    }
    const uint32_t rr = row < n ? row : (n - 1u);
    const float4* xr = reinterpret_cast<const float4*>(A.X + (size_t)rr * DP + FQ * q);
#pragma unroll
    for (int u = 0; u < FQ / 4; ++u) B.x[u] = xr[u];
    if constexpr (!LIST) {
      B.xn = A.xnorm[rr];
      if constexpr (MODE == 1) B.old = A.labels[rr];
    }
  };

  auto decide = [&](bool act0, uint32_t cnt, const uint32_t* sl, const float4* xv, int32_t& lab1, int32_t& lab2,
                    uint32_t& kind, uint32_t& ws, float& ubw, float& lbo) {
    auto partial = [&](uint32_t slot) {
      const float4* cp = TG ? reinterpret_cast<const float4*>(A.cft + slot * CS + FQ * q)
                            : reinterpret_cast<const float4*>(sCf + slot * CS + FQ * q);
      f32x2 acc = {0.0f, 0.0f};
#pragma unroll
      for (int u = 0; u < FQ / 4; ++u) {
        const float4 c = cp[u];
        const float4 x = xv[u];
        const f32x2 d0 = f32x2{x.x, x.y} - f32x2{c.x, c.y};
        const f32x2 d1 = f32x2{x.z, x.w} - f32x2{c.z, c.w};
        acc = __builtin_elementwise_fma(d0, d0, acc);
        acc = __builtin_elementwise_fma(d1, d1, acc);
      }
      return acc.x + acc.y;
    };
    uint32_t s1 = sl[0], s2 = sl[0];
    float U1 = FLT_MAX, L1 = FLT_MAX, Lo = FLT_MAX;
    auto take = [&](bool act, float Dt, uint32_t slot) {
      const bool tiny = !(Dt >= 0x1p-96f);
      const float r = __builtin_amdgcn_sqrtf(tiny ? 0x1p-96f : Dt);
      const float U = fmaf(r, 1.0f + 32.0f * U24, gam) * (1.0f + 4.0f * U24);
      const float L = fmaf(tiny ? 0.0f : r, 1.0f - 32.0f * U24, -gam) * (1.0f - 4.0f * U24);
      const bool w = act && U < U1;
      const float Lc = w ? L1 : L;
      const uint32_t sc = w ? s1 : slot;
      const bool lo = act && Lc < Lo;
      Lo = lo ? Lc : Lo;
      s2 = lo ? sc : s2;
      U1 = w ? U : U1;
      L1 = w ? L : L1;
      s1 = w ? slot : s1;
    };
    {
      const uint32_t sa = act0 ? sl[0] : 0u, sb = act0 ? sl[1] : 0u;
      const float pa = partial(sa), pb = partial(sb);
      take(act0, quad_sum(pa), sa);
      take(act0, quad_sum(pb), sb);
    }
#pragma unroll
    for (int r = 2; r < S1_LMAX; ++r) {
      const bool act = act0 && (uint32_t)r < cnt;
      if (__ballot(act) == 0ull) break;
      const uint32_t slot = act ? sl[r] : 0u;
      take(act, quad_sum(partial(slot)), slot);
    }
    const int32_t l1 = sPerm[s1], l2 = sPerm[s2];
    uint32_t kd = 2u;
    if (l1 >= 0) {
      if (Lo > U1)
        kd = 0u;
      else if (cnt == 2u && l2 >= 0 && s2 != s1)
        kd = 1u;
    }
    if (act0) {
      lab1 = l1;
      lab2 = l2;
      kind = kd;
      ws = s1;
      ubw = U1;
      lbo = Lo;
    }
  };
  auto emit = [&](bool act, uint32_t row, uint32_t kind, int32_t lab1, int32_t lab2, int32_t old) {
    const bool decided = act && kind == 0u;
    if constexpr (MODE == 0) {
      (void)old;
      if (decided && q == 0) A.labels[row] = lab1;
    } else {
      const bool changed = decided && lab1 != old && q == 0;
      const uint64_t mc = __ballot(changed);
      if (mc) {
        if (changed) {
          A.labels[row] = lab1;
          wc[cc + (uint32_t)__popcll(mc & ((1ull << lane) - 1ull))] =
              make_uint2(row, ((uint32_t)old << 16) | (uint32_t)lab1);
        }
        cc += (uint32_t)__popcll(mc);
      }
    }
    const bool enq = act && kind != 0u && q == 0;
    const uint64_t mq = __ballot(enq);
    if (mq) {
      const uint64_t m1 = __ballot(enq && kind == 1u);
      const uint64_t m2 = mq & ~m1;
      const uint64_t below = (1ull << lane) - 1ull;
      if (enq) {
        QEntry qe;
        qe.row = row;
        qe.i1 = kind == 1u ? (uint32_t)lab1 : 0u;
        qe.i2 = kind == 1u ? (uint32_t)lab2 : 0u;
        qe.kind = kind;
        const uint32_t pos = (kind == 1u) ? qn + (uint32_t)__popcll(m1 & below)
                                          : A.seg - 1u - (qf + (uint32_t)__popcll(m2 & below));
        wq[pos] = qe;
      }
      qn += (uint32_t)__popcll(m1);
      qf += (uint32_t)__popcll(m2);
    }
  };
  uint32_t rc = 0;
  auto rescore = [&](uint32_t nb) {
    if constexpr (BATCH) {
      const bool act = (uint32_t)c16 < nb;
      const uint32_t slot = act ? (uint32_t)c16 : 0u;
      const uint4 mt = sRm[wave * S1_RING + slot];
      float4 xv[FQ / 4];
      const float4* xs = reinterpret_cast<const float4*>(sRx + (wave * S1_RING + slot) * DP + FQ * q);
#pragma unroll
      for (int u = 0; u < FQ / 4; ++u) xv[u] = xs[u];
      const uint32_t cnt = mt.y >> 16;
      uint32_t sl[S1_LMAX];
      sl[0] = mt.z;
#pragma unroll
      for (int r = 1; r < S1_LMAX; ++r) sl[r] = 0u;
      {
        const float4* hp = sRh + ((wave * S1_RING + slot) * 4 + q) * 2;
        const float4 h0 = hp[0], h1 = hp[1];
        const float hv[8] = {h0.x, h0.y, h0.z, h0.w, h1.x, h1.y, h1.z, h1.w};
        float prev = u2f(mt.w);
#pragma unroll
        for (int r = 1; r < S1_LMAX; ++r) {
          if (__ballot(act && (uint32_t)r < cnt) == 0ull) break;
          float nl = FLT_MAX;
#pragma unroll
          for (int i = 0; i < 8; ++i) nl = min_raw(nl, hv[i] > prev ? hv[i] : FLT_MAX);
          prev = quad_min(nl);
          sl[r] = (uint32_t)r < cnt ? (f2u(prev) & SLOTM) : 0u;
        }
      }
      int32_t lab1 = 0, lab2 = 0;
      uint32_t kind = 2u, ws = 0u;
      float ubw = 0.0f, lbo = 0.0f;
      decide(act, cnt, sl, xv, lab1, lab2, kind, ws, ubw, lbo);
      emit(act, mt.x, kind, lab1, lab2, (int32_t)(mt.y & 0xFFFFu));
      resid(act && kind == 0u, ws, xv);
      if constexpr (MARG) {
        if (act && q == 0)
          A.marg[mt.x] = (kind == 0u && gscale)
                             ? s1g_base(s1g_margin(fminf(lbo, sRl[wave * S1_RING + slot]), ubw), sAd[lab1])
                             : 0.0f;
      }
    } else {
      (void)nb;
    }
  };

  auto tail = [&](uint32_t tile, const Buf& B, const float (&h)[2][4], float h2m) {
    uint32_t row;
    uint32_t lold = 0u;
    if constexpr (LIST) {
      row = wpick(wg0.x, wsub);
      lold = wpick(wg0.y, wsub);
    } else {
      row = tmap(tile) * 16u + (uint32_t)c16;
    }
    const bool valid = row < n;
    float hk[2][4];
#pragma unroll
    for (int cb = 0; cb < 2; ++cb)
#pragma unroll
      for (int i = 0; i < 4; ++i) hk[cb][i] = u2f(f2u(h[cb][i]) | qbits | ((uint32_t)(16 * cb + i) << MB));

    auto mn = [](float a, float b) { return __builtin_fminf(a, b); };
    auto mx = [](float a, float b) { return __builtin_fmaxf(a, b); };
    float la = FLT_MAX, lb = FLT_MAX;
    if constexpr (BATCH) {
      la = min3_raw(min3_raw(hk[0][0], hk[0][1], hk[0][2]), min3_raw(hk[0][3], hk[1][0], hk[1][1]),
                    min3_raw(hk[1][2], hk[1][3], FLT_MAX));
      la = quad_min(la);
    } else {
#pragma unroll
      for (int cb = 0; cb < 2; ++cb)
#pragma unroll
        for (int i = 0; i < 4; ++i) {
          lb = __builtin_amdgcn_fmed3f(la, lb, hk[cb][i]);
          la = mn(la, hk[cb][i]);
        }
      auto p = __builtin_amdgcn_permlane16_swap(f2u(la), f2u(la), false, false);
      auto p2 = __builtin_amdgcn_permlane16_swap(f2u(lb), f2u(lb), false, false);
      float a0 = u2f(p[0]), a1 = u2f(p[1]), b0 = u2f(p2[0]), b1 = u2f(p2[1]);
      la = mn(a0, a1);
      lb = mn(mx(a0, a1), mn(b0, b1));
      p = __builtin_amdgcn_permlane32_swap(f2u(la), f2u(la), false, false);
      p2 = __builtin_amdgcn_permlane32_swap(f2u(lb), f2u(lb), false, false);
      a0 = u2f(p[0]), a1 = u2f(p[1]), b0 = u2f(p2[0]), b1 = u2f(p2[1]);
      la = mn(a0, a1);
      lb = mn(mx(a0, a1), mn(b0, b1));
    }
    const float m = la;
#if KM_S1_ABL == 1
    if (valid && q == 0) A.labels[row] = sPerm[f2u(la) & SLOTM] + (h2m < -1e30f ? 1 : 0);
    return;
#endif
    float xq = 0.0f;
    if constexpr (MARG) {
      float xs = 0.0f;
#pragma unroll
      for (int u = 0; u < FQ / 4; ++u) {
        xs = fmaf(B.x[u].x, B.x[u].x, xs);
        xs = fmaf(B.x[u].y, B.x[u].y, xs);
        xs = fmaf(B.x[u].z, B.x[u].z, xs);
        xs = fmaf(B.x[u].w, B.x[u].w, xs);
      }
      xq = quad_sum(xs);
    }
    float xn;
    if constexpr (LIST)
      xn = s1g_xnorm(xq);
    else
      xn = B.xn;
    const float E = fmaf(e1, xn, e0);
    const bool bad = !(m >= -3.0e38f && m <= 3.0e38f) || !(xn <= 3.0e38f);
    constexpr float RP = RHO * (1.0f + 2.0f * RHO);
    const float R = m + RP * fabsf(m) + 2.0f * E;
    constexpr float IP = (1.0f / (1.0f - RP)) * (1.0f + 2.0f * U24);
    constexpr float IM = (1.0f / (1.0f + RP)) * (1.0f - 2.0f * U24);
    float T = R * (R >= 0.0f ? IP : IM);
    T = T * (T >= 0.0f ? (1.0f + 4.0f * U24) : (1.0f - 4.0f * U24));
    uint32_t cl = (h2m <= T) ? 0x10000u : 0u;
#pragma unroll
    for (int cb = 0; cb < 2; ++cb)
#pragma unroll
      for (int i = 0; i < 4; ++i) cl += (hk[cb][i] <= T) ? 1u : 0u;
    const uint32_t cq = bad ? 0u : quad_add_u(cl);
    const uint32_t cnt = cq & 0xFFFFu;
    const bool ovf = (cq >> 16) != 0u;

    const uint32_t sm = f2u(la) & SLOTM;
    const bool ok = valid && !bad && !ovf;
    const bool needy = ok && cnt >= 2u && cnt <= (uint32_t)S1_LMAX;
    const int32_t labm = sPerm[sm];
    const bool dec1 = ok && cnt == 1u && labm >= 0;
    int32_t old = 0;
    if constexpr (LIST)
      old = (int32_t)min(lold, (uint32_t)(A.k - 1));
    else if constexpr (MODE == 1)
      old = (int32_t)min((uint32_t)B.old, (uint32_t)(A.k - 1));
#if KM_S1_ABL == 2
    emit(valid, row, dec1 || needy ? 0u : 2u, labm, 0, old);
    return;
#endif
    float lbT = 0.0f;
    if constexpr (MARG) {
      const S1GRow gr = s1g_row(s, E, xq);
      float nl = h2m;
#pragma unroll
      for (int cb = 0; cb < 2; ++cb)
#pragma unroll
        for (int i = 0; i < 4; ++i) nl = min_raw(nl, hk[cb][i] > m ? hk[cb][i] : FLT_MAX);
      const float h2 = quad_min(nl);
      lbT = s1g_lb(T, RP, gr);
      if (valid && !needy && q == 0)
        A.marg[row] =
            (dec1 && gscale) ? s1g_base(s1g_margin(s1g_lb(h2, RP, gr), s1g_ub(m, RP, gr)), sAd[labm]) : 0.0f;
    }
    if constexpr (BATCH) {
      emit(valid && !needy, row, dec1 ? 0u : 2u, labm, 0, old);
      resid(dec1, sm, B.x);
      const uint64_t mrow = __ballot(needy && q == 0);
      if (mrow) {
        const uint32_t nn = (uint32_t)__popcll(mrow);
        const uint32_t rk = (uint32_t)__popcll(mrow & ((1ull << c16) - 1ull));
        const uint32_t space = (uint32_t)S1_RING - rc;
        const uint4 meta = make_uint4(row, (uint32_t)old | (cnt << 16), sm, f2u(la));
        auto stash = [&](uint32_t slot) {
          float4* xs = reinterpret_cast<float4*>(sRx + (wave * S1_RING + slot) * DP + FQ * q);
#pragma unroll
          for (int u = 0; u < FQ / 4; ++u) xs[u] = B.x[u];
          if (q == 0) sRm[wave * S1_RING + slot] = meta;
          float4* hp = sRh + ((wave * S1_RING + slot) * 4 + q) * 2;
          hp[0] = make_float4(hk[0][0], hk[0][1], hk[0][2], hk[0][3]);
          hp[1] = make_float4(hk[1][0], hk[1][1], hk[1][2], hk[1][3]);
          if constexpr (MARG)
            if (q == 0) sRl[wave * S1_RING + slot] = lbT;
        };
        constexpr bool EARLY0 = !SSE;
        if (EARLY0 && needy && rk < space) stash(rc + rk);
        if (nn >= space) {
          const S1RingSlot rs = s1_ring_slot((uint32_t)S1_RING, rc, nn, rk);
          const uint32_t full = s1_ring_batch((uint32_t)S1_RING, rc + nn);
          if constexpr (EARLY0) {
            for (uint32_t b = 1u;; ++b) {
              rescore((uint32_t)S1_RING);
              if (needy && rs.batch == b) stash(rs.slot);
              if (b == full) break;
            }
          } else {
            for (uint32_t b = 0u;; ++b) {
              if (needy && rs.batch == b) stash(rs.slot);
              if (b == full) break;
              rescore((uint32_t)S1_RING);
            }
          }
          rc = rs.rc;
        } else {
          if (!EARLY0 && needy) stash(rc + rk);
          rc += nn;
        }
      }
    } else {
      uint32_t sl[S1_LMAX];
      sl[0] = sm;
      sl[1] = f2u(lb) & SLOTM;
      float prev = lb;
      float ubw = 0.0f, lbo = 0.0f;
      (void)ubw;
      (void)lbo;
#pragma unroll
      for (int r = 2; r < S1_LMAX; ++r) {
        sl[r] = 0u;
        if (__ballot(needy && (uint32_t)r < cnt) == 0ull) continue;
        float nl = FLT_MAX;
#pragma unroll
        for (int cb = 0; cb < 2; ++cb)
#pragma unroll
          for (int i = 0; i < 4; ++i) nl = min_raw(nl, hk[cb][i] > prev ? hk[cb][i] : FLT_MAX);
        prev = quad_min(nl);
        sl[r] = f2u(prev) & SLOTM;
      }
      int32_t lab1 = labm, lab2 = 0;
      uint32_t kind = dec1 ? 0u : 2u, ws = sm;
      if (__ballot(needy) != 0ull) decide(needy, cnt, sl, B.x, lab1, lab2, kind, ws, ubw, lbo);
      emit(valid, row, kind, lab1, lab2, old);
      resid(valid && kind == 0u, ws, B.x);
    }
  };

  constexpr int TT = s1_tiles(NS2);
  auto process = [&](uint32_t st, const Buf (&BB)[TT]) {
    f16x8 bx[TT][NS2];
#pragma unroll
    for (int u = 0; u < TT; ++u)
#pragma unroll
      for (int t = 0; t < NS2; ++t) {
        const float4 a = BB[u].x[2 * t], c = BB[u].x[2 * t + 1];
        const f32x2 sv = {s, s};
        const f16x2 h0 = __builtin_convertvector(f32x2{a.x, a.y} * sv, f16x2);
        const f16x2 h1 = __builtin_convertvector(f32x2{a.z, a.w} * sv, f16x2);
        const f16x2 h2 = __builtin_convertvector(f32x2{c.x, c.y} * sv, f16x2);
        const f16x2 h3 = __builtin_convertvector(f32x2{c.z, c.w} * sv, f16x2);
        bx[u][t] = __builtin_shufflevector(__builtin_shufflevector(h0, h1, 0, 1, 2, 3),
                                           __builtin_shufflevector(h2, h3, 0, 1, 2, 3), 0, 1, 2, 3, 4, 5, 6, 7);
      }
    float h[TT][2][4], h2m[TT];
#pragma unroll
    for (int u = 0; u < TT; ++u) {
      h2m[u] = FLT_MAX;
#pragma unroll
      for (int cb = 0; cb < 2; ++cb)
#pragma unroll
        for (int i = 0; i < 4; ++i) h[u][cb][i] = FLT_MAX;
    }
    const float4* cnl = reinterpret_cast<const float4*>(sCn + 4 * q);
    struct Pair {
      f16x8 a[2][2][NS2];
      float4 c[2][2];
    };
    auto load_pair = [&](int blk, Pair& P) {
#pragma unroll
      for (int e = 0; e < 2; ++e)
#pragma unroll
        for (int cb = 0; cb < 2; ++cb) {
          P.c[e][cb] = cnl[8 * (blk + e) + 4 * cb];
#pragma unroll
          for (int t = 0; t < NS2; ++t)
            P.a[e][cb][t] = __builtin_bit_cast(f16x8, sImg[(((blk + e) * 2 + cb) * NS2 + t) * 64 + lane]);
        }
    };
    auto mfmas = [&](const Pair& P, f32x4 (&a)[TT][2][2]) {
#pragma unroll
      for (int u = 0; u < TT; ++u)
#pragma unroll
        for (int e = 0; e < 2; ++e)
#pragma unroll
          for (int cb = 0; cb < 2; ++cb)
            a[u][e][cb] = f32x4{P.c[e][cb].x, P.c[e][cb].y, P.c[e][cb].z, P.c[e][cb].w};
#pragma unroll
      for (int t = 0; t < NS2; ++t)
#pragma unroll
        for (int cb = 0; cb < 2; ++cb)
#pragma unroll
          for (int e = 0; e < 2; ++e)
#pragma unroll
            for (int u = 0; u < TT; ++u)
              a[u][e][cb] = __builtin_amdgcn_mfma_f32_16x16x32_f16(P.a[e][cb][t], bx[u][t], a[u][e][cb], 0, 0, 0);
    };
    auto keys = [&](int blk, const f32x4 (&a)[TT][2][2]) {
#pragma unroll
      for (int u = 0; u < TT; ++u) {
        float t[2][4];
#pragma unroll
        for (int cb = 0; cb < 2; ++cb)
#pragma unroll
          for (int i = 0; i < 4; ++i) {
            const float ka = u2f((f2u(a[u][0][cb][i]) & KMASK) | (uint32_t)blk);
            const float kb = u2f((f2u(a[u][1][cb][i]) & KMASK) | (uint32_t)(blk + 1));
            t[cb][i] = __builtin_amdgcn_fmed3f(h[u][cb][i], ka, kb);
            h[u][cb][i] = __builtin_fminf(__builtin_fminf(h[u][cb][i], ka), kb);
          }
        float m = h2m[u];
#pragma unroll
        for (int cb = 0; cb < 2; ++cb) {
          m = __builtin_fminf(__builtin_fminf(m, t[cb][0]), t[cb][1]);
          m = __builtin_fminf(__builtin_fminf(m, t[cb][2]), t[cb][3]);
        }
        h2m[u] = m;
      }
    };
    auto pin = [&]() {
#pragma unroll
      for (int u = 0; u < TT; ++u) {
        asm volatile("" : "+v"(h2m[u]));
#pragma unroll
        for (int cb = 0; cb < 2; ++cb)
#pragma unroll
          for (int i = 0; i < 4; ++i) asm volatile("" : "+v"(h[u][cb][i]));
      }
    };
    if constexpr (NB <= 8 && s1_waves(NS2, NB) == 12) {
      Pair P;
      load_pair(0, P);
#pragma unroll
      for (int blk = 0; blk < NB; blk += 2) {
        f32x4 a[TT][2][2];
        mfmas(P, a);
        __builtin_amdgcn_sched_barrier(0);
        if (blk + 2 < NB) load_pair(blk + 2, P);
        __builtin_amdgcn_sched_barrier(0);
        keys(blk, a);
        pin();
        __builtin_amdgcn_sched_barrier(0);
      }
    } else if constexpr (NB <= 8) {
      Pair pr[2];
      load_pair(0, pr[0]);
#pragma unroll
      for (int blk = 0; blk < NB; blk += 2) {
        const Pair& P = pr[(blk >> 1) & 1];
        if (blk + 2 < NB) load_pair(blk + 2, pr[((blk >> 1) + 1) & 1]);
        f32x4 a[TT][2][2];
        mfmas(P, a);
        keys(blk, a);
        __builtin_amdgcn_sched_barrier(0);
      }
    } else {
      static_assert(NB % 4 == 0, "NB > 8 must be a multiple of 4");
      Pair pr[2];
      load_pair(0, pr[0]);
#pragma unroll 1
      for (int blk = 0; blk < NB; blk += 4) {
        f32x4 a[TT][2][2];
        load_pair(blk + 2, pr[1]);
        mfmas(pr[0], a);
        keys(blk, a);
        __builtin_amdgcn_sched_barrier(0);
        if (blk + 4 < NB) load_pair(blk + 4, pr[0]);
        mfmas(pr[1], a);
        keys(blk + 2, a);
        __builtin_amdgcn_sched_barrier(0);
      }
    }
#pragma unroll
    for (int u = 0; u < TT; ++u) tail(st * TT + (uint32_t)u, BB[u], h[u], h2m[u]);
  };

  constexpr int NBUF = LIST ? 2 : KM_S1_NBUF > 0 ? KM_S1_NBUF : (NS2 == 1 && NB > 8 && S1_WAVES == 8 ? 3 : 2);
  static_assert(!LIST || TT == 1, "the gated instance walks its list one tile per step");
  const uint32_t nst = LIST ? (wln + 15u) / 16u : (ntiles + (uint32_t)TT - 1u) / (uint32_t)TT;
  const uint32_t st0 = LIST ? 0u : gw, sw = LIST ? 1u : nw;
  Buf b[NBUF][TT];
  auto load_step = [&](uint32_t st, Buf (&BB)[TT]) {
#pragma unroll
    for (int u = 0; u < TT; ++u) load(st * TT + (uint32_t)u, BB[u]);
  };
  if constexpr (LIST) {
    static_assert(NBUF == 2 && TT == 1, "the list walk alternates two row buffers");
    load(0u, b[0][0]);
    for (uint32_t g = 0u; g * 4u < nst; ++g) {
      wg2 = wfetch(g + 2u);
      bool done = false;
#pragma unroll
      for (int i = 0; i < 4; ++i) {
        if (!done) {
          load((uint32_t)(i + 1), b[(i + 1) & 1][0]);
          __builtin_amdgcn_sched_barrier(0);
          wsub = (uint32_t)i;
          process(g * 4u + (uint32_t)i, b[i & 1]);
          done = g * 4u + (uint32_t)(i + 1) >= nst;
        }
      }
      if (done) break;
      wg0 = wg1;
      wg1 = wmark(g + 2u, wg2);
    }
  } else {
#pragma unroll
    for (int u = 0; u + 1 < NBUF; ++u) load_step(st0 + (uint32_t)u * sw, b[u]);
    for (uint32_t st = st0; st < nst; st += (uint32_t)NBUF * sw) {
      bool done = false;
#pragma unroll
      for (int u = 0; u < NBUF; ++u) {
        if (!done) {
          load_step(st + (uint32_t)(u + NBUF - 1) * sw, b[(u + NBUF - 1) % NBUF]);
          process(st + (uint32_t)u * sw, b[u]);
          done = st + (uint32_t)(u + 1) * sw >= nst;
        }
      }
      if (done) break;
    }
  }
  if (rc) rescore(rc);
  if (lane == 0) {
    A.qcount[2 * gw] = qn;
    A.qcount[2 * gw + 1] = qf;
    if constexpr (MODE == 1) A.chg_cnt[gw] = cc;
  }
  if constexpr (SSE) {
#pragma unroll
    for (int o = 32; o >= 1; o >>= 1) ssa += __shfl_xor(ssa, o);
    if (lane == 0 && ssa != 0.0) atomicAdd(A.sse, ssa);
  }
}

__global__ __launch_bounds__(1024) void k_s1_shift(const double* __restrict__ C, double* __restrict__ cref, int k,
                                                   int d, double* __restrict__ acc,
                                                   float* __restrict__ accud, int reset,
                                                   const int* __restrict__ gate) {
  if (*gate) return;
  __shared__ float sv[1024];
  __shared__ float stop[3];
  const int lane = threadIdx.x & 63, wave = threadIdx.x >> 6, nwv = blockDim.x >> 6;
  for (int j = wave; j < k; j += nwv) {
    double sh = 0.0;
    for (int f = lane; f < d; f += 64) {
      const double a = C[(size_t)j * d + f];
      const double df = a - cref[(size_t)j * d + f];
      sh = fma(df, df, sh);
      cref[(size_t)j * d + f] = a;
    }
#pragma unroll
    for (int o = 32; o >= 1; o >>= 1) sh += __shfl_xor(sh, o);
    if (lane == 0) sv[j] = s1g_shift(sh);
  }
  __syncthreads();
  if (wave == 0) {
    float m1 = -1.0f, m2 = -1.0f;
    int a1 = 0;
    for (int j = lane; j < k; j += 64) {
      const float v = sv[j];
      m2 = v > m1 ? m1 : fmaxf(m2, v);
      a1 = v > m1 ? j : a1;
      m1 = v > m1 ? v : m1;
    }
#pragma unroll
    for (int o = 32; o >= 1; o >>= 1) {
      const float om1 = __shfl_xor(m1, o), om2 = __shfl_xor(m2, o);
      const int oa1 = __shfl_xor(a1, o);
      m2 = fmaxf(fminf(m1, om1), fmaxf(m2, om2));
      a1 = om1 > m1 ? oa1 : a1;
      m1 = fmaxf(m1, om1);
    }
    if (lane == 0) {
      stop[0] = m1;
      stop[1] = fmaxf(m2, 0.0f);
      stop[2] = __int_as_float(a1);
    }
  }
  __syncthreads();
  {
    const float top1 = stop[0], top2 = stop[1];
    const int atop = __float_as_int(stop[2]);
    for (int j = threadIdx.x; j < k; j += blockDim.x) {
      float up, dn;
      acc[j] = s1g_acc_pass(acc[j], sv[j], j == atop ? top2 : top1, top1, reset != 0, &up, &dn);
      accud[j] = up;
      accud[k + j] = dn;
    }
  }
}

struct S1GateArgs {
  const int32_t* labels;
  const float* marg;
  int64_t n;
  int k;
  uint32_t seg;
  const float* acc_up;
  uint2* wl;
  uint32_t* wl_cnt;
  int init;
  const int32_t* init_dev;
  const int* gate;
};

constexpr int S1G_UNITS = 2;
constexpr uint32_t S1G_TRIP = 256u * S1G_UNITS;

template <int WAVES>
__global__ __launch_bounds__(WAVES * 64) void k_s1_gate(S1GateArgs A) {
  if (*A.gate) return;
  __shared__ float sUp[1024];
  for (int i = threadIdx.x; i < A.k; i += WAVES * 64) sUp[i] = A.acc_up[i];
  __syncthreads();
  const int lane = threadIdx.x & 63, wave = threadIdx.x >> 6;
  const uint32_t gw = blockIdx.x * WAVES + wave;
  const uint64_t n = (uint64_t)A.n;
  const uint64_t r0 = (uint64_t)gw * A.seg, r1 = max(r0, min(n, r0 + A.seg));
  uint2* wl = A.wl + (size_t)gw * A.seg;
  const uint64_t below = (1ull << lane) - 1ull;
  const bool init = A.init != 0 || (A.init_dev && *A.init_dev != 0);
  const uint32_t km1 = (uint32_t)(A.k - 1);
  uint32_t cnt = 0;
  struct Trip {
    int4 lab[S1G_UNITS];
    float4 bs[S1G_UNITS];
  };
  auto fetch = [&](uint64_t base, Trip& T) {
#pragma unroll
    for (int u = 0; u < S1G_UNITS; ++u) {
      const uint64_t row = base + 256u * u + 4u * (uint32_t)lane;
      T.lab[u] = *reinterpret_cast<const int4*>(A.labels + row);
      T.bs[u] = init ? make_float4(0.0f, 0.0f, 0.0f, 0.0f) : *reinterpret_cast<const float4*>(A.marg + row);
    }
  };
  auto fetch_tail = [&](uint64_t base, Trip& T) {
#pragma unroll
    for (int u = 0; u < S1G_UNITS; ++u) {
      const uint64_t row = base + 256u * u + 4u * (uint32_t)lane;
      int32_t l[4];
      float b[4];
#pragma unroll
      for (int i = 0; i < 4; ++i) {
        const bool in = row + i < r1;
        l[i] = in ? A.labels[row + i] : 0;
        b[i] = (in && !init) ? A.marg[row + i] : 0.0f;
      }
      T.lab[u] = make_int4(l[0], l[1], l[2], l[3]);
      T.bs[u] = make_float4(b[0], b[1], b[2], b[3]);
    }
  };
  auto sift = [&](uint64_t base, const Trip& T) {
#pragma unroll
    for (int u = 0; u < S1G_UNITS; ++u) {
      const uint64_t row = base + 256u * u + 4u * (uint32_t)lane;
      auto clampk = [&](int32_t v) -> uint32_t { return (uint32_t)v < km1 ? (uint32_t)v : km1; };
      const uint32_t l[4] = {clampk(T.lab[u].x), clampk(T.lab[u].y), clampk(T.lab[u].z), clampk(T.lab[u].w)};
      const float b[4] = {T.bs[u].x, T.bs[u].y, T.bs[u].z, T.bs[u].w};
      bool ls[4];
      uint32_t c = 0;
#pragma unroll
      for (int i = 0; i < 4; ++i) {
        ls[i] = row + i < r1 && (init || !s1g_keep(b[i], sUp[l[i]]));
        c += ls[i] ? 1u : 0u;
      }
      const uint64_t b0 = __ballot((c & 1u) != 0u), b1 = __ballot((c & 2u) != 0u), b2 = __ballot((c & 4u) != 0u);
      if ((b0 | b1 | b2) == 0ull) continue;
      uint32_t pos = cnt + (uint32_t)__popcll(b0 & below) + 2u * (uint32_t)__popcll(b1 & below) +
                     4u * (uint32_t)__popcll(b2 & below);
#pragma unroll
      for (int i = 0; i < 4; ++i)
        if (ls[i]) wl[pos++] = make_uint2((uint32_t)(row + i), l[i]);
      cnt += (uint32_t)__popcll(b0) + 2u * (uint32_t)__popcll(b1) + 4u * (uint32_t)__popcll(b2);
    }
  };
  const uint64_t rfull = r0 + (r1 - r0) / S1G_TRIP * S1G_TRIP;
  uint64_t base = r0;
  if (base < rfull) {
    Trip ta, tb;
    fetch(base, ta);
    tb = ta;
    for (;;) {
      if (base + S1G_TRIP < rfull) fetch(base + S1G_TRIP, tb);
      sift(base, ta);
      base += S1G_TRIP;
      if (base >= rfull) break;
      if (base + S1G_TRIP < rfull) fetch(base + S1G_TRIP, ta);
      sift(base, tb);
      base += S1G_TRIP;
      if (base >= rfull) break;
    }
  }
  if (base < r1) {
    Trip tt;
    fetch_tail(base, tt);
    sift(base, tt);
  }
  if (lane == 0) A.wl_cnt[gw] = cnt;
}

__global__ __launch_bounds__(256) void k_s1_apply(double* __restrict__ stats, double* __restrict__ full, int64_t len,
                                                  int mode, const int* __restrict__ gate) {
  if (*gate) return;
  const int64_t i = (int64_t)blockIdx.x * blockDim.x + threadIdx.x;
  if (i >= len) return;
  double v = stats[i];
  if (mode >= 1 && i != len - 1) v = full[i] + v;
  full[i] = v;
  stats[i] = mode == 2 ? 0.0 : v;
}

#ifndef KM_S1D_MIN
#define KM_S1D_MIN 256
#endif
constexpr uint32_t S1D_MIN = KM_S1D_MIN;
constexpr int S1D_ROWS = 8;
__global__ __launch_bounds__(1024) void k_s1_delta(const float* __restrict__ X, int dp, int d, int k,
                                                   const uint2* __restrict__ chg, const uint32_t* __restrict__ cnt,
                                                   const uint32_t* __restrict__ qcount, int nw, uint32_t seg, int kr,
                                                   int nr, double* __restrict__ stats,
                                                   const int* __restrict__ gate) {
  if (*gate) return;
  extern __shared__ double smem_d[];
  const int d1 = d + 1;
  double* tab = smem_d;
  uint32_t* pre = reinterpret_cast<uint32_t*>(smem_d + (size_t)kr * d1);
  const int lane = threadIdx.x & 63, wave = threadIdx.x >> 6, nwv = blockDim.x >> 6;
  {
    uint32_t* wsum = pre + nw + 1;
    auto total = [&](int w) {
      uint32_t v = cnt[w];
      if (qcount) v += qcount[2 * w] + qcount[2 * w + 1];
      return min(v, seg);
    };
    const int nt = (int)blockDim.x, t = (int)threadIdx.x;
    const int c = (nw + nt - 1) / nt, b0 = t * c;
    uint32_t v = 0;
    for (int i = 0; i < c; ++i)
      if (b0 + i < nw) v += total(b0 + i);
    uint32_t inc = v;
#pragma unroll
    for (int o = 1; o < 64; o <<= 1) {
      const uint32_t u = __shfl_up(inc, o);
      inc += lane >= o ? u : 0u;
    }
    if (lane == 63) wsum[wave] = inc;
    __syncthreads();
    uint32_t base = 0;
    for (int i = 0; i < wave; ++i) base += wsum[i];
    uint32_t run = base + inc - v;
    for (int i = 0; i < c; ++i)
      if (b0 + i < nw) {
        pre[b0 + i] = run;
        run += total(b0 + i);
      }
    if (t == nt - 1) pre[nw] = run;
  }
  __syncthreads();
  const int r = (int)(blockIdx.x % (uint32_t)nr);
  const uint32_t ns = gridDim.x / (uint32_t)nr, sl = blockIdx.x / (uint32_t)nr;
  const uint32_t nc = pre[nw];
  const uint32_t lo = (uint32_t)r * (uint32_t)kr;
  const uint32_t span = min((uint32_t)kr, (uint32_t)k - lo);
  const uint32_t per = max(max(S1D_MIN, (uint32_t)kr * (uint32_t)d1 / 16u), (nc + ns - 1u) / ns);
  const uint32_t e0 = sl * per;
  if (sl >= ns || e0 >= nc) return;
  const uint32_t e1 = min(nc, e0 + per);
  for (int i = threadIdx.x; i < (int)span * d1; i += blockDim.x) tab[i] = 0.0;
  __syncthreads();
  int sgl = 0;
  {
    const uint32_t e = min(e0 + (uint32_t)wave * 64u + (uint32_t)lane, nc - 1u);
    int h = nw - 1;
    while (sgl < h) {
      const int mid = (sgl + h + 1) >> 1;
      if (pre[mid] <= e) sgl = mid; else h = mid - 1;
    }
  }
  auto at = [&](uint32_t e) {
    while (sgl + 1 < nw && pre[sgl + 1] <= e) ++sgl;
    return chg[(size_t)sgl * seg + (e - pre[sgl])];
  };
  for (uint32_t base = e0 + (uint32_t)wave * 64u; base < e1; base += (uint32_t)nwv * 64u) {
    const uint32_t e = base + (uint32_t)lane;
    const uint2 c = e < e1 ? at(e) : make_uint2(0u, 0u);
    const uint32_t o = c.y >> 16, nn = c.y & 0xFFFFu;
    const bool mine = e < e1 && o != nn && (o - lo < span || nn - lo < span);
    uint64_t m = __ballot(mine);
    while (m) {
      uint32_t row[S1D_ROWS], oy[S1D_ROWS];
      int na = 0;
#pragma unroll
      for (int j = 0; j < S1D_ROWS; ++j) {
        row[j] = 0u;
        oy[j] = 0u;
        if (m) {
          const int src = __builtin_ctzll(m);
          m &= m - 1ull;
          row[j] = (uint32_t)__builtin_amdgcn_readlane((int)c.x, src);
          oy[j] = (uint32_t)__builtin_amdgcn_readlane((int)c.y, src);
          ++na;
        }
      }
      for (int f0 = 0; f0 < d; f0 += 64) {
        const int f = f0 + lane;
        float x[S1D_ROWS];
#pragma unroll
        for (int j = 0; j < S1D_ROWS; ++j) x[j] = (j < na && f < d) ? X[(size_t)row[j] * dp + f] : 0.0f;
        if (f < d)
#pragma unroll
          for (int j = 0; j < S1D_ROWS; ++j) {
            const uint32_t jo = oy[j] >> 16, jn = oy[j] & 0xFFFFu;
            if (j >= na) continue;
            if (jo - lo < span) atomicAdd(tab + (size_t)(jo - lo) * d1 + f, -(double)x[j]);
            if (jn - lo < span) atomicAdd(tab + (size_t)(jn - lo) * d1 + f, (double)x[j]);
          }
      }
      if (lane < na) {
        uint32_t jy = 0u;
#pragma unroll
        for (int j = 0; j < S1D_ROWS; ++j) jy = lane == j ? oy[j] : jy;
        const uint32_t jo = jy >> 16, jn = jy & 0xFFFFu;
        if (jo - lo < span) atomicAdd(tab + (size_t)(jo - lo) * d1 + d, -1.0);
        if (jn - lo < span) atomicAdd(tab + (size_t)(jn - lo) * d1 + d, 1.0);
      }
    }
  }
  __syncthreads();
  for (int i = threadIdx.x; i < (int)span * d1; i += blockDim.x) {
    const double v = tab[i];
    if (v != 0.0) atomicAdd(stats + (size_t)lo * d1 + i, v);
  }
}

static int s1_geo_waves(const Geometry& g) { return s1_waves(g.dp / 32, g.kp / 32); }
static int64_t s1_grid(const Geometry& g, int n_cu, int* nbk, uint32_t* seg) {
  const int tt = s1_tiles(g.dp / 32);
  const int w = s1_geo_waves(g);
  const int64_t nst = ((g.n + 15) / 16 + tt - 1) / tt;
  int64_t blocks = n_cu;
  if (blocks > (nst + w - 1) / w) blocks = (nst + w - 1) / w;
  *nbk = (int)blocks;
  const int64_t nw = blocks * w;
  *seg = nw ? (uint32_t)(((nst + nw - 1) / nw) * 16 * tt) : 0u;
  return nw;
}

size_t s1_chg_entries(const Geometry& g, int n_cu) {
  int nbk;
  uint32_t seg;
  const int64_t nw = s1_grid(g, n_cu, &nbk, &seg);
  return (size_t)std::max<int64_t>(nw * (int64_t)seg, 1);
}

size_t s1_wave_slots(int n_cu) { return (size_t)n_cu * S1_MAX_WAVES; }

bool s1_delta_ok(const Geometry& g, int n_cu) {
  (void)n_cu;
  return g.k <= 65535;
}

hipError_t launch_chg_delta(const float* X, const Geometry& g, const uint2* chg, const uint32_t* chg_cnt, int nw,
                            uint32_t seg, double* stats, int n_cu, const int* gate, hipStream_t s,
                            const uint32_t* qcount) {
  if (g.n == 0 || nw == 0) return hipSuccess;
  if (g.k > 65535) return hipErrorInvalidValue;
  constexpr size_t LDS = 160 * 1024;
  const size_t pre = ((size_t)nw + 1 + 16) * 4;
  const size_t row = (size_t)(g.d + 1) * 8;
  if (pre > 64 * 1024 || pre + row > LDS) return hipErrorInvalidValue;
  const int kmax = (int)((LDS - pre) / row);
  const int nr = (g.k + kmax - 1) / kmax;
  const int kr = (g.k + nr - 1) / nr;
  const int ns = std::max(1, (n_cu + nr / 2) / nr);
  hipLaunchKernelGGL(k_s1_delta, dim3((unsigned)(nr * ns)), dim3(1024), (size_t)kr * row + pre, s, X, g.dp, g.d, g.k,
                     chg, chg_cnt, qcount, nw, seg, kr, nr, stats, gate);
  return hipGetLastError();
}

hipError_t launch_s1_delta(const float* X, const Geometry& g, const uint2* chg, const uint32_t* chg_cnt,
                           double* stats, int n_cu, const int* gate, hipStream_t s, const uint32_t* qcount) {
  if (g.n == 0) return hipSuccess;
  int nbk;
  uint32_t seg;
  const int64_t nw = s1_grid(g, n_cu, &nbk, &seg);
  if (!s1_delta_ok(g, n_cu)) return hipErrorInvalidValue;
  return launch_chg_delta(X, g, chg, chg_cnt, (int)nw, seg, stats, n_cu, gate, s, qcount);
}

hipError_t launch_s1_apply(double* stats, double* full, int64_t len, int mode, const int* gate, hipStream_t s) {
  if (len <= 0) return hipSuccess;
  hipLaunchKernelGGL(k_s1_apply, dim3((unsigned)((len + 255) / 256)), dim3(256), 0, s, stats, full, len, mode, gate);
  return hipGetLastError();
}

bool s1_ok(const Geometry& g) {
  if (g.dp % 32 || g.kp % 64) return false;
  switch ((g.dp / 32) * 100 + g.kp / 32) {
    case 202: case 204: case 206: case 208:
    case 102: case 104: case 106: case 108: case 112: case 116: case 132:
    case 216:
    case 402: case 404:
      return true;
    default:
      return false;
  }
}

static S1Geo s1_geo(const Geometry& g) {
  S1Geo sg;
  sg.nb = g.kp / 32;
  sg.mb = ceil_log2_c(sg.nb);
  sg.ns2 = g.dp / 32;
  return sg;
}

size_t s1_table_entries(const Geometry& g) { return (size_t)32 << s1_geo(g).mb; }

hipError_t launch_s1_color(const float* C32, const Geometry& g, int32_t* perm, const int* gate, hipStream_t s) {
  const S1Geo sg = s1_geo(g);
  if (g.k > (g.dp == 32 ? 1024 : 512)) return hipErrorInvalidValue;
  switch (g.dp) {
    case 32:
      if (g.k > 512)
        hipLaunchKernelGGL((k_s1_color<32, 1024>), dim3(1), dim3(1024), 0, s, C32, g.k, g.dp, sg.nb, sg.mb, perm, gate);
      else
        hipLaunchKernelGGL((k_s1_color<32, 512>), dim3(1), dim3(512), 0, s, C32, g.k, g.dp, sg.nb, sg.mb, perm, gate);
      break;
    case 64:
      hipLaunchKernelGGL((k_s1_color<64, 512>), dim3(1), dim3(512), 0, s, C32, g.k, g.dp, sg.nb, sg.mb, perm, gate);
      break;
    case 128:
      hipLaunchKernelGGL((k_s1_color<128, 512>), dim3(1), dim3(512), 0, s, C32, g.k, g.dp, sg.nb, sg.mb, perm, gate);
      break;
    default: return hipErrorInvalidValue;
  }
  return hipGetLastError();
}

hipError_t launch_s1_prep(const double* C64, const float* C32, const Geometry& g, const int32_t* perm,
                          const float* cmax, const float* xabs, const float* cabs, float* cft, float* cn2o,
                          uint4* img, float* cst, const int* gate, hipStream_t s) {
  const S1Geo sg = s1_geo(g);
  const int nt = 32 << sg.mb;
  hipLaunchKernelGGL(k_s1_prep, dim3(nt + 1), dim3(64), 0, s, C64, C32, g.k, g.d, g.dp, sg, perm, cmax, xabs, cabs,
                     cft, cn2o, img, cst, gate);
  return hipGetLastError();
}

template <int NS2, int NB>
static void launch_s1_gated(int nbk, size_t lds, hipStream_t s, const S1Args& a, bool dense) {
  if constexpr (s1_gated(NS2, NB)) {
    if (dense)
      KM_TIMED_LAUNCH((k_s1<NS2, NB, 1, false, false, 2>), dim3(nbk), dim3(s1_waves(NS2, NB) * 64),
                      lds + s1_gate_lds(NS2, NB), s, a);
    else
      KM_TIMED_LAUNCH((k_s1<NS2, NB, 1, false, false, 1>), dim3(nbk), dim3(s1_waves(NS2, NB) * 64),
                      lds + s1_gate_lds(NS2, NB), s, a);
  }
}

bool s1_gate_ok(const Geometry& g) {
  if (!s1_ok(g) || g.k > 1024) return false;
  const int ns2 = g.dp / 32, nb = g.kp / 32;
  switch (ns2 * 100 + nb) {
    case 202: case 204: case 206: case 208:
    case 102: case 104: case 106: case 108: case 112: case 116:
      return s1_gated(ns2, nb);
    default:
      return false;
  }
}

hipError_t launch_s1_gate(const Geometry& g, const double* C64, const int32_t* labels, const S1GateBufs& b, int init,
                          const int32_t* init_dev, int n_cu, const int* gate, hipStream_t s) {
  if (g.n == 0) return hipSuccess;
  if (!s1_gate_ok(g)) return hipErrorInvalidValue;
  int nbk;
  uint32_t seg;
  (void)s1_grid(g, n_cu, &nbk, &seg);
  hipLaunchKernelGGL(k_s1_shift, dim3(1), dim3(1024), 0, s, C64, b.cref, g.k, g.d, b.acc, b.accud,
                     init == 2 ? 1 : 0, gate);
  hipError_t e = hipGetLastError();
  if (e != hipSuccess) return e;
  if (init == 2) return hipSuccess;
  S1GateArgs a{labels, b.marg, g.n, g.k, seg, b.accud, b.wl, b.wl_cnt, init, init_dev, gate};
  if (s1_geo_waves(g) == 12)
    hipLaunchKernelGGL(k_s1_gate<12>, dim3(nbk), dim3(12 * 64), 0, s, a);
  else
    hipLaunchKernelGGL(k_s1_gate<8>, dim3(nbk), dim3(8 * 64), 0, s, a);
  return hipGetLastError();
}

hipError_t launch_s1(const float* X, const float* xnorm, const Geometry& g, const uint4* img, const float* cn2o,
                     const float* cft, const int32_t* perm, const float* cst, int32_t* labels,
                     QEntry* queue, uint32_t* qcount, uint2* chg, uint32_t* chg_cnt, int delta, int n_cu,
                     QLayout* ql, const int* gate, hipStream_t s, int rev, double* sse, const S1GateBufs* gt,
                     int gdense) {
  ql->seg = 0;
  ql->nwaves = 0;
  if (g.n == 0) return hipSuccess;
  const S1Geo sg = s1_geo(g);
  const int nt = 32 << sg.mb;
  int nbk;
  uint32_t seg;
  const int64_t nw = s1_grid(g, n_cu, &nbk, &seg);
  ql->seg = seg;
  ql->nwaves = (uint32_t)nw;
  if (sse && !delta) return hipErrorInvalidValue;
  S1Args a{X, xnorm, g.n, g.k, g.d, seg, img, cn2o, cft, perm, cst, labels, queue, qcount, chg, chg_cnt, sse, gate,
           gt ? gt->wl : nullptr, gt ? gt->wl_cnt : nullptr, gt ? gt->marg : nullptr,
           gt ? gt->accud + g.k : nullptr};
  if (gt && (!delta || sse || !s1_gate_ok(g))) return hipErrorInvalidValue;
  const size_t lds = s1_lds_bytes(sg.ns2, sg.nb, !s1_table_global(sg.ns2, sg.nb));
  if (lds > 160 * 1024) return hipErrorInvalidValue;
  (void)nt;
#define KM_S1_CASE(NS2_, NB_)                                                                                   \
  case NS2_ * 100 + NB_:                                                                                        \
    if (gt)                                                                                                     \
      launch_s1_gated<NS2_, NB_>(nbk, lds, s, a, gdense != 0);                                                             \
    else if (delta && sse)                                                                                      \
      KM_TIMED_LAUNCH((k_s1<NS2_, NB_, 1, false, true>), dim3(nbk), dim3(s1_waves(NS2_, NB_) * 64), lds, s, a); \
    else if (delta && rev && KM_S1_SERP && NS2_ == 2 && NB_ == 8)                                               \
      KM_TIMED_LAUNCH((k_s1<2, 8, 1, true>), dim3(nbk), dim3(s1_waves(2, 8) * 64), lds, s, a);                  \
    else if (delta)                                                                                             \
      KM_TIMED_LAUNCH((k_s1<NS2_, NB_, 1>), dim3(nbk), dim3(s1_waves(NS2_, NB_) * 64), lds, s, a);              \
    else                                                                                                        \
      KM_TIMED_LAUNCH((k_s1<NS2_, NB_, 0>), dim3(nbk), dim3(s1_waves(NS2_, NB_) * 64), lds, s, a);              \
    break;
  switch (sg.ns2 * 100 + sg.nb) {
    KM_S1_CASE(2, 2) KM_S1_CASE(2, 4) KM_S1_CASE(2, 6) KM_S1_CASE(2, 8)
    KM_S1_CASE(1, 2) KM_S1_CASE(1, 4) KM_S1_CASE(1, 6) KM_S1_CASE(1, 8) KM_S1_CASE(1, 12) KM_S1_CASE(1, 16)
    KM_S1_CASE(1, 32) KM_S1_CASE(2, 16) KM_S1_CASE(4, 2) KM_S1_CASE(4, 4)
    default:
      return hipErrorInvalidValue;
  }
#undef KM_S1_CASE
  return hipGetLastError();
}

}
```

assignment--2-group7-distributed-k-means_amd/engine.py:

```python
from __future__ import annotations

import ctypes
from typing import Optional, Tuple

import numpy as np

from . import _lib

_PD = ctypes.POINTER(ctypes.c_double)
_PF = ctypes.POINTER(ctypes.c_float)
_PI32 = ctypes.POINTER(ctypes.c_int32)
_PI64 = ctypes.POINTER(ctypes.c_int64)


def _ptr(a: np.ndarray, t):
    return a.ctypes.data_as(t)


class HipEngine:

    def __init__(self, device: int = 0, distributed: bool = False):
        self.lib = _lib.load()
        n = _lib.device_count()
        if n <= 0:
            raise _lib.KmError("no HIP device visible: the MI355X path needs a gfx950 GPU")
        self.device = device
        ctx = ctypes.c_void_p()
        _lib.check(self.lib.km_create(device, ctypes.byref(ctx)), "km_create")
        self.ctx = ctx
        self.n = 0
        self.d = 0
        self.k = 0
        self._stats_t = None
        self.weighted = False
        self._tstream = None
        self._rep_mode, self._rep_t = 0, None
        self._coll_ev = None
        self.distributed = distributed
        if distributed:
            import torch
            self._torch = torch
            self._tstream = torch.cuda.Stream(device=f"cuda:{device}")
            _lib.check(self.lib.km_set_stream(self.ctx, ctypes.c_void_p(self._tstream.cuda_stream)), "km_set_stream")

    def close(self):
        if getattr(self, "ctx", None) is not None and self.ctx.value:
            self.lib.km_destroy(self.ctx)
            self.ctx = ctypes.c_void_p()

    def __del__(self):
        try:
            self.close()
        except Exception:
            pass

    def _c(self, rc, what):
        return _lib.check(rc, what)

    def load_host(self, rows: np.ndarray) -> int:
        rows = np.ascontiguousarray(rows, dtype=np.float32)
        if rows.ndim != 2:
            raise ValueError("rows must be a 2-D array")
        n, d = rows.shape
        self._c(self.lib.km_load_begin(self.ctx, n, d), "km_load_begin")
        if n:
            self._c(self.lib.km_load_rows(self.ctx, 0, _ptr(rows, _PF), n), "km_load_rows")
        self.n, self.d = n, d
        self.weighted = False
        self._stats_t = None
        self._rep_mode, self._rep_t = 0, None
        return n

    def load_weights(self, w) -> None:
        was = self.weighted
        if w is None:
            self._c(self.lib.km_clear_weights(self.ctx), "km_clear_weights")
            self.weighted = False
        else:
            w = np.ascontiguousarray(w, dtype=np.float64)
            if w.shape != (self.n,):
                raise ValueError(f"weights of shape {w.shape} for {self.n} local rows")
            self._c(self.lib.km_set_weights(self.ctx, 0, _ptr(w, _PD), self.n), "km_set_weights")
            self.weighted = True
        if was != self.weighted and self._stats_t is not None:
            self._stats_t = None
            if self.k:
                self._bind_stats()

    def load_blobs(self, n: int, d: int, global_row0: int, n_centers: int, box: float = 10.0, std: float = 1.0,
                   seed: int = 0) -> int:
        self._c(self.lib.km_generate_blobs(self.ctx, n, d, global_row0, n_centers, box, std, seed),
                "km_generate_blobs")
        self.n, self.d = n, d
        self.weighted = False
        self._stats_t = None
        self._rep_mode, self._rep_t = 0, None
        return n

    def sum_x(self) -> np.ndarray:
        out = np.zeros(self.d, dtype=np.float64)
        self._c(self.lib.km_sum_x(self.ctx, _ptr(out, _PD)), "km_sum_x")
        return out

    def set_sse(self, enable: bool) -> None:
        self._c(self.lib.km_set_sse(self.ctx, 1 if enable else 0), "km_set_sse")

    def set_screen(self, mode: int) -> None:
        self._c(self.lib.km_set_screen(self.ctx, int(mode)), "km_set_screen")

    def screen(self) -> int:
        m = ctypes.c_int32()
        self._c(self.lib.km_get_screen(self.ctx, ctypes.byref(m)), "km_get_screen")
        return m.value

    def set_centroids(self, C: np.ndarray) -> None:
        C = np.ascontiguousarray(C, dtype=np.float64)
        k, d = C.shape
        self._c(self.lib.km_set_centroids(self.ctx, _ptr(C, _PD), k, d), "km_set_centroids")
        rebind = self.distributed and (self._stats_t is None or k != self.k)
        self.k = k
        if rebind:
            self._bind_stats()

    def stats_len(self) -> int:
        return self.k * (self.d + 1) + 1 + (self.k if self.weighted else 0)

    def _bind_stats(self) -> None:
        torch = self._torch
        self._stats_t = torch.zeros(self.stats_len(), dtype=torch.float64, device=f"cuda:{self.device}")
        torch.cuda.synchronize(self.device)
        self._c(self.lib.km_bind_stats_buffer(self.ctx, ctypes.c_void_p(self._stats_t.data_ptr())),
                "km_bind_stats_buffer")

    def get_centroids(self, which: int = 0) -> np.ndarray:
        out = np.empty((self.k, self.d), dtype=np.float64)
        self._c(self.lib.km_get_centroids(self.ctx, which, _ptr(out, _PD)), "km_get_centroids")
        return out

    def assign_stats(self) -> None:
        self._c(self.lib.km_assign_stats(self.ctx), "km_assign_stats")

    def run_collective(self, fn, tensor=None) -> None:
        with self._torch.cuda.stream(self._tstream):
            if self._coll_ev is not None:
                e0 = self._torch.cuda.Event(enable_timing=True)
                e1 = self._torch.cuda.Event(enable_timing=True)
                e0.record(self._tstream)
            work = fn(self._stats_t if tensor is None else tensor, async_op=True)
            if work is not None:
                work.wait()
            if self._coll_ev is not None:
                e1.record(self._tstream)
                self._coll_ev.append((e0, e1))

    def time_collectives(self, enable: bool) -> None:
        self._coll_ev = [] if enable else None

    def collective_ms(self) -> Tuple[float, int]:
        evs = self._coll_ev or []
        if evs:
            self._torch.cuda.synchronize(self.device)
        return sum(a.elapsed_time(b) for a, b in evs), len(evs)

    def update(self) -> Tuple[_lib.KmStatus, np.ndarray]:
        st = _lib.KmStatus()
        counts = np.zeros(self.k, dtype=np.int64)
        self._c(self.lib.km_update(self.ctx, ctypes.byref(st), _ptr(counts, _PI64)), "km_update")
        return st, counts

    def batch_begin(self) -> None:
        self._c(self.lib.km_batch_begin(self.ctx), "km_batch_begin")

    def update_async(self, tol: float, empty_seed: int = 0) -> None:
        self._c(self.lib.km_update_async(self.ctx, float(tol), int(empty_seed)), "km_update_async")

    def set_layout(self, sizes, row0: int, device_repair: int) -> None:
        sizes = np.ascontiguousarray(sizes, dtype=np.int64)
        self._c(self.lib.km_set_layout(self.ctx, _ptr(sizes, _PI64), len(sizes), int(row0), int(device_repair)),
                "km_set_layout")
        self._rep_mode = int(device_repair)
        self._rep_t = None

    def repair_state(self) -> Tuple[bool, bool]:
        a, w = ctypes.c_int32(), ctypes.c_int32()
        self._c(self.lib.km_repair_state(self.ctx, ctypes.byref(a), ctypes.byref(w)), "km_repair_state")
        return bool(a.value), bool(w.value)

    def repair_bind(self) -> None:
        if self._rep_t is None or self._rep_t.numel() != self.k * self.d:
            torch = self._torch
            self._rep_t = torch.zeros(self.k * self.d, dtype=torch.float64, device=f"cuda:{self.device}")
            torch.cuda.synchronize(self.device)
            self._c(self.lib.km_bind_repair_buffer(self.ctx, ctypes.c_void_p(self._rep_t.data_ptr())),
                    "km_bind_repair_buffer")

    def repair_exchange(self, allreduce) -> None:
        self.run_collective(allreduce, self._rep_t)
        self._c(self.lib.km_repair_apply_async(self.ctx), "km_repair_apply_async")

    def batch_end(self, m: int):
        st = (_lib.KmStatus * max(m, 1))()
        counts = np.zeros((max(m, 1), self.k), dtype=np.int64)
        n = ctypes.c_int32(0)
        self._c(self.lib.km_batch_end(self.ctx, st, _ptr(counts, _PI64), ctypes.byref(n)), "km_batch_end")
        return [(st[i], counts[i]) for i in range(n.value)]

    def replace_rows(self, ids, rows: np.ndarray) -> None:
        ids = np.ascontiguousarray(ids, dtype=np.int32)
        rows = np.ascontiguousarray(rows, dtype=np.float64).reshape(len(ids), self.d)
        if len(ids):
            self._c(self.lib.km_replace_rows(self.ctx, _ptr(ids, _PI32), _ptr(rows, _PD), len(ids)),
                    "km_replace_rows")

    def commit(self) -> None:
        self._c(self.lib.km_commit(self.ctx), "km_commit")

    def gather_rows(self, local_idx) -> np.ndarray:
        idx = np.ascontiguousarray(local_idx, dtype=np.int64)
        out = np.empty((len(idx), self.d), dtype=np.float64)
        if len(idx):
            self._c(self.lib.km_gather_rows(self.ctx, _ptr(idx, _PI64), len(idx), _ptr(out, _PD)),
                    "km_gather_rows")
        return out

    def bernoulli(self, seeds, sizes, bases, fraction: float) -> Optional[np.ndarray]:
        seeds = np.ascontiguousarray(seeds, dtype=np.uint64)
        sizes = np.ascontiguousarray(sizes, dtype=np.int64)
        bases = np.ascontiguousarray(bases, dtype=np.int64)
        cap = int(4.0 * fraction * float(sizes.sum())) + 64 * max(len(sizes), 1)
        out = np.empty(cap, dtype=np.int64)
        n = ctypes.c_int64(0)
        rc = self.lib.km_bernoulli_sample(self.ctx, seeds.ctypes.data_as(ctypes.POINTER(ctypes.c_uint64)),
                                          _ptr(sizes, _PI64), _ptr(bases, _PI64), len(sizes), float(fraction),
                                          _ptr(out, _PI64), cap, ctypes.byref(n))
        if rc == -1:
            return None
        self._c(rc, "km_bernoulli_sample")
        return out[:n.value].copy()

    def seed_begin(self) -> None:
        self._c(self.lib.km_seed_begin(self.ctx), "km_seed_begin")

    def seed_update(self, first_id: int) -> float:
        phi = ctypes.c_double(0.0)
        self._c(self.lib.km_seed_update(self.ctx, int(first_id), ctypes.byref(phi)), "km_seed_update")
        return phi.value

    def seed_sample(self, seed: int, rnd: int, global_row0: int, ell: float, phi: float,
                    cap: Optional[int] = None) -> Optional[np.ndarray]:
        cap = int(4.0 * ell) + 64 if cap is None else int(cap)
        out = np.empty(max(cap, 1), dtype=np.int64)
        n = ctypes.c_int64(0)
        rc = self.lib.km_seed_sample(self.ctx, ctypes.c_uint64(int(seed) & (2 ** 64 - 1)), int(rnd), int(global_row0),
                                     float(ell), float(phi), _ptr(out, _PI64), cap, ctypes.byref(n))
        if rc == -1:
            return None
        self._c(rc, "km_seed_sample")
        return out[:n.value].copy()

    def seed_weights(self, m_total: int) -> np.ndarray:
        out = np.zeros(int(m_total), dtype=np.int64)
        self._c(self.lib.km_seed_weights(self.ctx, int(m_total), _ptr(out, _PI64)), "km_seed_weights")
        return out

    def seed_read(self) -> Tuple[np.ndarray, np.ndarray]:
        d2 = np.empty(self.n, dtype=np.float64)
        near = np.empty(self.n, dtype=np.int32)
        self._c(self.lib.km_seed_read(self.ctx, _ptr(d2, _PD), _ptr(near, _PI32)), "km_seed_read")
        return d2, near

    def seed_end(self) -> None:
        self._c(self.lib.km_seed_end(self.ctx), "km_seed_end")

    def predict(self) -> np.ndarray:
        out = np.empty(self.n, dtype=np.int32)
        self._c(self.lib.km_predict(self.ctx, _ptr(out, _PI32)), "km_predict")
        return out

    def predict_device(self) -> None:
        self._c(self.lib.km_predict(self.ctx, None), "km_predict")

    def labels(self) -> np.ndarray:
        out = np.empty(self.n, dtype=np.int32)
        self._c(self.lib.km_labels(self.ctx, _ptr(out, _PI32)), "km_labels")
        return out

    def sync(self) -> None:
        self._c(self.lib.km_sync(self.ctx), "km_sync")

    def info(self) -> dict:
        inf = _lib.KmInfo()
        self._c(self.lib.km_info_get(self.ctx, ctypes.byref(inf)), "km_info_get")
        out = {f: getattr(inf, f) for f, _ in inf._fields_}
        rows = ctypes.c_int64(-1)
        self._c(self.lib.km_gated_rows(self.ctx, ctypes.byref(rows)), "km_gated_rows")
        out["gated_rows"] = rows.value
        v = [ctypes.c_int32() for _ in range(5)]
        if self.lib.km_stats_route(self.ctx, *[ctypes.byref(x) for x in v]) == 0:
            for key, x in zip(("stats_route", "stats_cluster_ranges", "stats_kr", "stats_feature_ranges", "stats_fr"), v):
                out[key] = x.value
        return out

    _PHASES = {"assign": 0, "resolve": 1, "stats": 2, "update": 3, "prep": 4, "seed": 5}

    def profile(self, enable: bool = True, phases=None, every: int = 1) -> None:
        mask = 0
        if enable:
            mask = -1 if phases is None else sum(1 << self._PHASES[p] for p in phases)
        self._c(self.lib.km_profile_every(self.ctx, int(every)), "km_profile_every")
        self._c(self.lib.km_profile(self.ctx, mask), "km_profile")

    def prof_read(self, kind: str) -> Tuple[float, int]:
        ms = ctypes.c_double()
        n = ctypes.c_int64()
        self._c(self.lib.km_prof_read(self.ctx, _lib.KERNEL_KINDS[kind], ctypes.byref(ms), ctypes.byref(n)),
                "km_prof_read")
        return ms.value, n.value


def make_engine(comm, device: Optional[int] = None) -> HipEngine:
    if device is None:
        n = _lib.device_count()
        dev = comm.local_rank % n if n > 0 else comm.local_rank
    else:
        dev = device
    return HipEngine(dev, distributed=comm.world > 1)
```

include/kmeans_amd.h:

```cpp
#ifndef KMEANS_AMD_H
#define KMEANS_AMD_H

#include <stdint.h>

#ifdef __cplusplus
extern "C" {
#endif

#define KM_ABI_VERSION 6

#define KM_OK 0
#define KM_EMPTY 1
#define KM_ERR_ARG (-1)
#define KM_ERR_HIP (-2)
#define KM_ERR_STATE (-3)
#define KM_ERR_UNSUPPORTED (-4)

typedef struct km_ctx km_ctx;

typedef struct km_status {
  double sse;
  double max_shift;
  int32_t n_empty;
  int32_t nonfinite;
  int32_t q_rerank;
  int32_t q_full;
  int32_t ran;
  int32_t stop_reason;
  int32_t repaired;
  int32_t reserved;
} km_status;

#define KM_STOP_CONVERGED 1
#define KM_STOP_EMPTY 2
#define KM_STOP_NONFINITE 3
#define KM_MAX_BATCH 32

typedef struct km_info {
  int64_t n;
  int32_t d, dp;
  int32_t k, kp;
  int32_t path;
  int32_t n_cu;
  int32_t device;
  int32_t fused_stats;
  int32_t delta_stats;
} km_info;

#define KM_K_ASSIGN 0
#define KM_K_RESOLVE 1
#define KM_K_STATS 2
#define KM_K_UPDATE 3
#define KM_K_PREP 4
#define KM_K_SEED 5
#define KM_K_COUNT 6

int km_abi_version(void);
const char* km_last_error(void);
int km_device_count(int* out);

int km_create(int device, km_ctx** out);
int km_destroy(km_ctx* ctx);
int km_set_stream(km_ctx* ctx, void* hip_stream);
int km_sync(km_ctx* ctx);
int km_info_get(km_ctx* ctx, km_info* out);
int km_gated_rows(km_ctx* ctx, int64_t* out);
int km_stats_route(km_ctx* ctx, int32_t* route, int32_t* cluster_ranges, int32_t* kr, int32_t* feature_ranges,
                   int32_t* fr);

int km_load_begin(km_ctx* ctx, int64_t n, int32_t d);
int km_load_rows(km_ctx* ctx, int64_t row0, const float* rows, int64_t nrows);
int km_generate_blobs(km_ctx* ctx, int64_t n, int32_t d, int64_t global_row0, int32_t n_centers, float box,
                      float stddev, uint64_t seed);
int km_set_weights(km_ctx* ctx, int64_t row0, const double* w, int64_t nrows);
int km_clear_weights(km_ctx* ctx);
int km_sum_x(km_ctx* ctx, double* out_d);
int km_set_sse(km_ctx* ctx, int32_t enable);

int km_set_centroids(km_ctx* ctx, const double* C, int32_t k, int32_t d);
int km_get_centroids(km_ctx* ctx, int32_t which, double* out);

int km_assign_stats(km_ctx* ctx);
int km_stats_buffer(km_ctx* ctx, void** dev_ptr, int64_t* len);
int km_bind_stats_buffer(km_ctx* ctx, void* dev_ptr);

int km_update(km_ctx* ctx, km_status* st, int64_t* counts);
int km_set_layout(km_ctx* ctx, const int64_t* sizes, int32_t nparts, int64_t row0, int32_t device_repair);
int km_repair_state(km_ctx* ctx, int32_t* armed, int32_t* waiting);
int km_repair_buffer(km_ctx* ctx, void** buffer, int64_t* len);
int km_bind_repair_buffer(km_ctx* ctx, void* buffer);
int km_repair_apply_async(km_ctx* ctx);
int km_batch_begin(km_ctx* ctx);
int km_update_async(km_ctx* ctx, double tol, int64_t empty_seed);
int km_batch_end(km_ctx* ctx, km_status* st, int64_t* counts, int32_t* n_ran);
int km_replace_rows(km_ctx* ctx, const int32_t* cluster_ids, const double* rows, int32_t n);
int km_commit(km_ctx* ctx);

int km_gather_rows(km_ctx* ctx, const int64_t* local_idx, int32_t n, double* out);

int km_bernoulli_sample(km_ctx* ctx, const uint64_t* seeds, const int64_t* sizes, const int64_t* bases,
                        int32_t nparts, double fraction, int64_t* out, int64_t cap, int64_t* n_out);

int km_predict(km_ctx* ctx, int32_t* labels_out);
int km_labels(km_ctx* ctx, int32_t* labels_out);

int km_seed_begin(km_ctx* ctx);
int km_seed_update(km_ctx* ctx, int32_t first_id, double* phi_local);
int km_seed_sample(km_ctx* ctx, uint64_t seed, int32_t round, int64_t global_row0, double ell, double phi,
                   int64_t* out, int64_t cap, int64_t* n_out);
int km_seed_weights(km_ctx* ctx, int32_t m_total, int64_t* counts_out);
int km_seed_read(km_ctx* ctx, double* d2_out, int32_t* near_out);
int km_seed_end(km_ctx* ctx);

#define KM_SCREEN_AUTO (-1)
#define KM_SCREEN_S1 4
#define KM_SCREEN_ONE 5
int km_set_screen(km_ctx* ctx, int32_t mode);
int km_get_screen(km_ctx* ctx, int32_t* mode);

int km_profile(km_ctx* ctx, int32_t enable);
int km_profile_every(km_ctx* ctx, int32_t period);
int km_prof_read(km_ctx* ctx, int32_t kind, double* total_ms, int64_t* launches);

#ifdef __cplusplus
}
#endif
#endif
```

Measured before the change: 1235 Lloyd it/s.

## Add pairwise-bound gate path resolving ambiguous rows with two-centroid check

Result: no change. 1227 Lloyd it/s (-0.7%).

```diff
diff --git a/assignment--2-group7-distributed-k-means_amd/_lib.py b/assignment--2-group7-distributed-k-means_amd/_lib.py
--- a/assignment--2-group7-distributed-k-means_amd/_lib.py
+++ b/assignment--2-group7-distributed-k-means_amd/_lib.py
@@ -55,6 +55,7 @@
     "km_sync": [_P],
     "km_info_get": [_P, ctypes.POINTER(KmInfo)],
     "km_gated_rows": [_P, _PI64],
+    "km_pair_rows": [_P, _PI64],
     "km_stats_route": [_P, _PI32, _PI32, _PI32, _PI32, _PI32],
     "km_load_begin": [_P, _I64, _I32],
     "km_load_rows": [_P, _I64, _PF, _I64],
diff --git a/assignment--2-group7-distributed-k-means_amd/csrc/km_internal.h b/assignment--2-group7-distributed-k-means_amd/csrc/km_internal.h
--- a/assignment--2-group7-distributed-k-means_amd/csrc/km_internal.h
+++ b/assignment--2-group7-distributed-k-means_amd/csrc/km_internal.h
@@ -168,10 +168,14 @@
   double* cref;
   double* acc;
   float* accud;
+  uint32_t* pair_cnt;
 };
 bool s1_gate_ok(const Geometry& g);
 hipError_t launch_s1_gate(const Geometry& g, const double* C64, const int32_t* labels, const S1GateBufs& b, int init,
                           const int32_t* init_dev, int n_cu, const int* gate, hipStream_t s);
+hipError_t launch_s1_pair(const float* X, const float* C32, const float* cst, const Geometry& g, int32_t* labels,
+                          QEntry* queue, uint32_t* qcount, uint2* chg, uint32_t* chg_cnt, const S1GateBufs& b, int n_cu,
+                          const int* gate, hipStream_t s);
 size_t s1_chg_entries(const Geometry& g, int n_cu);
 size_t s1_wave_slots(int n_cu);
 bool s1_delta_ok(const Geometry& g, int n_cu);
diff --git a/assignment--2-group7-distributed-k-means_amd/csrc/km_runtime.hip b/assignment--2-group7-distributed-k-means_amd/csrc/km_runtime.hip
--- a/assignment--2-group7-distributed-k-means_amd/csrc/km_runtime.hip
+++ b/assignment--2-group7-distributed-k-means_amd/csrc/km_runtime.hip
@@ -85,7 +85,7 @@
   uint2* chg = nullptr;
   uint32_t* chg_cnt = nullptr;
   bool delta_ready = false;
-  km::S1GateBufs gt{nullptr, nullptr, nullptr, nullptr, nullptr, nullptr};
+  km::S1GateBufs gt{nullptr, nullptr, nullptr, nullptr, nullptr, nullptr, nullptr};
   bool bounds_valid = false;
   bool last_gated = false;
   uint32_t gated_nw = 0;
@@ -268,6 +268,7 @@
   dfree(c->gt.marg);
   dfree(c->gt.wl);
   dfree(c->gt.wl_cnt);
+  c->gt.pair_cnt = nullptr;
   dfree(c->gt.cref);
   dfree(c->gt.acc);
   dfree(c->gt.accud);
@@ -570,13 +571,15 @@
       if (!c->gt.marg) {
         KM_HIP(hipMalloc(&c->gt.marg, sizeof(float) * (size_t)g.n));
         KM_HIP(hipMalloc(&c->gt.wl, sizeof(uint2) * km::s1_chg_entries(g, c->n_cu)));
-        KM_HIP(hipMalloc(&c->gt.wl_cnt, sizeof(uint32_t) * km::s1_wave_slots(c->n_cu)));
+        KM_HIP(hipMalloc(&c->gt.wl_cnt, sizeof(uint32_t) * 2 * km::s1_wave_slots(c->n_cu)));
+        KM_HIP(hipMemsetAsync(c->gt.wl_cnt, 0, sizeof(uint32_t) * 2 * km::s1_wave_slots(c->n_cu), c->stream));
+        c->gt.pair_cnt = c->gt.wl_cnt + km::s1_wave_slots(c->n_cu);
         KM_HIP(hipMalloc(&c->gt.cref, sizeof(double) * (size_t)g.k * g.d));
         KM_HIP(hipMemsetAsync(c->gt.cref, 0, sizeof(double) * (size_t)g.k * g.d, c->stream));
         KM_HIP(hipMalloc(&c->gt.acc, sizeof(double) * (size_t)g.k));
-        KM_HIP(hipMalloc(&c->gt.accud, sizeof(float) * 2 * (size_t)g.k));
+        KM_HIP(hipMalloc(&c->gt.accud, sizeof(float) * (3 * (size_t)g.k + 1)));
         KM_HIP(hipMemsetAsync(c->gt.acc, 0, sizeof(double) * (size_t)g.k, c->stream));
-        KM_HIP(hipMemsetAsync(c->gt.accud, 0, sizeof(float) * 2 * (size_t)g.k, c->stream));
+        KM_HIP(hipMemsetAsync(c->gt.accud, 0, sizeof(float) * (3 * (size_t)g.k + 1), c->stream));
       }
       gdense = !bounds_were_valid;
       ProfScope ps(c, KM_K_PREP);
@@ -590,6 +593,9 @@
                            c->labels, c->queue, c->qcount, c->chg, c->chg_cnt, with_stats ? 1 : 0, c->n_cu,
                            &c->ql, c->gate, c->stream, gated ? 0 : next_sweep(c), s1_sse,
                            gated ? &c->gt : nullptr, gdense ? 1 : 0));
+      if (gated && !gdense)
+        KM_HIP(km::launch_s1_pair(c->X, c->C32, c->s1_cst, g, c->labels, c->queue, c->qcount, c->chg, c->chg_cnt,
+                                  c->gt, c->n_cu, c->gate, c->stream));
     }
     if (gated) {
       c->bounds_valid = true;
@@ -826,8 +832,27 @@
     return KM_OK;
   }
   KM_HIP(hipSetDevice(c->device));
+  const size_t slots = km::s1_wave_slots(c->n_cu);
+  std::vector<uint32_t> cnt(2 * slots);
+  KM_HIP(hipMemcpyAsync(cnt.data(), c->gt.wl_cnt, sizeof(uint32_t) * cnt.size(), hipMemcpyDeviceToHost, c->stream));
+  KM_HIP(hipStreamSynchronize(c->stream));
+  int64_t total = 0;
+  for (uint32_t w = 0; w < c->gated_nw; ++w) total += (int64_t)cnt[w] + cnt[slots + w];
+  *out = total;
+  return KM_OK;
+}
+
+int km_pair_rows(km_ctx* c, int64_t* out) {
+  KM_REQUIRE(c && out, KM_ERR_ARG, "null arg");
+  *out = -1;
+  if (!c->last_gated || !c->gt.wl_cnt || c->gated_nw == 0) return KM_OK;
+  if (c->gated_dense) {
+    *out = 0;
+    return KM_OK;
+  }
+  KM_HIP(hipSetDevice(c->device));
   std::vector<uint32_t> cnt(c->gated_nw);
-  KM_HIP(hipMemcpyAsync(cnt.data(), c->gt.wl_cnt, sizeof(uint32_t) * cnt.size(), hipMemcpyDeviceToHost, c->stream));
+  KM_HIP(hipMemcpyAsync(cnt.data(), c->gt.pair_cnt, sizeof(uint32_t) * cnt.size(), hipMemcpyDeviceToHost, c->stream));
   KM_HIP(hipStreamSynchronize(c->stream));
   int64_t total = 0;
   for (uint32_t v : cnt) total += v;
diff --git a/assignment--2-group7-distributed-k-means_amd/csrc/km_s1_gate.h b/assignment--2-group7-distributed-k-means_amd/csrc/km_s1_gate.h
--- a/assignment--2-group7-distributed-k-means_amd/csrc/km_s1_gate.h
+++ b/assignment--2-group7-distributed-k-means_amd/csrc/km_s1_gate.h
@@ -100,6 +100,56 @@
 }
 KM_S1G_FN bool s1g_keep(float base, float acc_up) { return base > acc_up; }
 
+constexpr uint32_t S1G_PAIR_IDS = 1024u;
+
+KM_S1G_FN uint32_t s1g_bits(float v) {
+  uint32_t b;
+  __builtin_memcpy(&b, &v, 4);
+  return b;
+}
+KM_S1G_FN float s1g_float(uint32_t b) {
+  float v;
+  __builtin_memcpy(&v, &b, 4);
+  return v;
+}
+KM_S1G_FN float s1g_full(float base) { return base > 0.0f ? base : 0.0f; }
+KM_S1G_FN float s1g_pair_pack(float b3, uint32_t partner) {
+  if (!(b3 >= 0x1p-100f && b3 <= 3.0e38f) || partner >= S1G_PAIR_IDS) return 0.0f;
+  return s1g_float(0x80000000u | (s1g_bits(b3) & ~(S1G_PAIR_IDS - 1u)) | partner);
+}
+KM_S1G_FN bool s1g_is_pair(float base) { return base < 0.0f; }
+KM_S1G_FN float s1g_pair_b3(float base) { return s1g_float(s1g_bits(base) & 0x7FFFFC00u); }
+KM_S1G_FN uint32_t s1g_pair_partner(float base) { return s1g_bits(base) & (S1G_PAIR_IDS - 1u); }
+KM_S1G_FN bool s1g_pair_keep(float base, float acc_up) { return s1g_is_pair(base) && s1g_pair_b3(base) > acc_up; }
+
+struct S1GPair {
+  uint32_t w, o;
+  bool decided;
+  float base;
+};
+KM_S1G_FN S1GPair s1g_pair_eval(float b3, float acc_up_a, uint32_t a, uint32_t b, float La, float Ua, float Lb,
+                                float Ub, float dn_a, float dn_b, float st_a, float st_b, float thr) {
+  S1GPair r;
+  const bool wa = !(Ub < Ua);
+  r.w = wa ? a : b;
+  r.o = wa ? b : a;
+  const float Uw = wa ? Ua : Ub, Lo = wa ? Lb : La;
+  const float dn = wa ? dn_a : dn_b, st = wa ? st_a : st_b;
+  r.decided = Lo > Uw && Uw <= 3.0e38f && Lo <= 3.0e38f;
+  r.base = 0.0f;
+  if (!r.decided) return r;
+  const float M = s1g_dn(b3 - acc_up_a);
+  const float lb3 = s1g_dn(M + La);
+  const float full = s1g_margin(fminf(Lo, lb3), Uw);
+  const float fb = s1g_base(full, dn);
+  if (full > s1g_up(thr * st) && fb > 0.0f) {
+    r.base = fb;
+    return r;
+  }
+  r.base = s1g_pair_pack(s1g_base(s1g_margin(lb3, Uw), dn), r.o);
+  return r;
+}
+
 KM_S1G_FN float s1g_xnorm(float xs) {
   float v = s1g_up(xs * (1.0f + 64.0f * S1G_U));
   v = !(v < 0x1p-96f) ? v : 0x1p-96f;
diff --git a/assignment--2-group7-distributed-k-means_amd/csrc/km_screen1.hip b/assignment--2-group7-distributed-k-means_amd/csrc/km_screen1.hip
--- a/assignment--2-group7-distributed-k-means_amd/csrc/km_screen1.hip
+++ b/assignment--2-group7-distributed-k-means_amd/csrc/km_screen1.hip
@@ -59,6 +59,9 @@
 #ifndef KM_S1_GATE
 #define KM_S1_GATE 1
 #endif
+#ifndef KM_S1_PAIR
+#define KM_S1_PAIR 1
+#endif
 constexpr size_t s1_gate_ring_lds(int ns2, int nb) { return (size_t)s1_waves(ns2, nb) * s1_ring(ns2, nb) * 4; }
 constexpr size_t s1_gate_lds(int ns2, int nb) { return s1_gate_ring_lds(ns2, nb) + (size_t)32 * nb * 4; }
 constexpr bool s1_gated_with(int ns2, int nb, size_t extra) {
@@ -124,6 +127,26 @@
   (void)frexpf(m, &e);
   return ldexpf(1.0f, 14 - e);
 }
+
+template <int FQ>
+__device__ __forceinline__ float s1_partial(const float4* cp, const float4* xv) {
+  f32x2 acc = {0.0f, 0.0f};
+#pragma unroll
+  for (int u = 0; u < FQ / 4; ++u) {
+    const float4 c = cp[u];
+    const float4 x = xv[u];
+    const f32x2 d0 = f32x2{x.x, x.y} - f32x2{c.x, c.y};
+    const f32x2 d1 = f32x2{x.z, x.w} - f32x2{c.z, c.w};
+    acc = __builtin_elementwise_fma(d0, d0, acc);
+    acc = __builtin_elementwise_fma(d1, d1, acc);
+  }
+  return acc.x + acc.y;
+}
+#define S1_BOUNDS(Dt, gam, U, L)                                                             \
+  const bool tiny_##U = !((Dt) >= 0x1p-96f);                                                 \
+  const float r_##U = __builtin_amdgcn_sqrtf(tiny_##U ? 0x1p-96f : (Dt));                    \
+  const float U = fmaf(r_##U, 1.0f + 32.0f * U24, (gam)) * (1.0f + 4.0f * U24);              \
+  const float L = fmaf(tiny_##U ? 0.0f : r_##U, 1.0f - 32.0f * U24, -(gam)) * (1.0f - 4.0f * U24)
 
 }
 
@@ -359,6 +382,8 @@
   uint2 wg0 = make_uint2(0xFFFFFFFFu, 0u), wg1 = wg0, wg2 = wg0;
   uint32_t wsub = 0;
   const bool gscale = MARG && s1g_scale_ok(s);
+  float lthr = 0.0f;
+  if constexpr (MARG) lthr = A.acc_dn[2 * A.k];
   auto wfetch = [&](uint32_t g) { return wlp[min(g * 64u + (uint32_t)lane, A.seg - 1u)]; };
   auto wmark = [&](uint32_t g, uint2 v) {
     return make_uint2(g * 64u + (uint32_t)lane < wln ? v.x : 0xFFFFFFFFu, v.y);
@@ -396,25 +421,12 @@
     auto partial = [&](uint32_t slot) {
       const float4* cp = TG ? reinterpret_cast<const float4*>(A.cft + slot * CS + FQ * q)
                             : reinterpret_cast<const float4*>(sCf + slot * CS + FQ * q);
-      f32x2 acc = {0.0f, 0.0f};
-#pragma unroll
-      for (int u = 0; u < FQ / 4; ++u) {
-        const float4 c = cp[u];
-        const float4 x = xv[u];
-        const f32x2 d0 = f32x2{x.x, x.y} - f32x2{c.x, c.y};
-        const f32x2 d1 = f32x2{x.z, x.w} - f32x2{c.z, c.w};
-        acc = __builtin_elementwise_fma(d0, d0, acc);
-        acc = __builtin_elementwise_fma(d1, d1, acc);
-      }
-      return acc.x + acc.y;
+      return s1_partial<FQ>(cp, xv);
     };
     uint32_t s1 = sl[0], s2 = sl[0];
     float U1 = FLT_MAX, L1 = FLT_MAX, Lo = FLT_MAX;
     auto take = [&](bool act, float Dt, uint32_t slot) {
-      const bool tiny = !(Dt >= 0x1p-96f);
-      const float r = __builtin_amdgcn_sqrtf(tiny ? 0x1p-96f : Dt);
-      const float U = fmaf(r, 1.0f + 32.0f * U24, gam) * (1.0f + 4.0f * U24);
-      const float L = fmaf(tiny ? 0.0f : r, 1.0f - 32.0f * U24, -gam) * (1.0f - 4.0f * U24);
+      S1_BOUNDS(Dt, gam, U, L);
       const bool w = act && U < U1;
       const float Lc = w ? L1 : L;
       const uint32_t sc = w ? s1 : slot;
@@ -504,9 +516,10 @@
       for (int u = 0; u < FQ / 4; ++u) xv[u] = xs[u];
       const uint32_t cnt = mt.y >> 16;
       uint32_t sl[S1_LMAX];
-      sl[0] = mt.z;
+      sl[0] = MARG ? (mt.w & SLOTM) : mt.z;
 #pragma unroll
       for (int r = 1; r < S1_LMAX; ++r) sl[r] = 0u;
+      float key3 = FLT_MAX;
       {
         const float4* hp = sRh + ((wave * S1_RING + slot) * 4 + q) * 2;
         const float4 h0 = hp[0], h1 = hp[1];
@@ -520,6 +533,14 @@
           for (int i = 0; i < 8; ++i) nl = min_raw(nl, hv[i] > prev ? hv[i] : FLT_MAX);
           prev = quad_min(nl);
           sl[r] = (uint32_t)r < cnt ? (f2u(prev) & SLOTM) : 0u;
+          if constexpr (MARG && KM_S1_PAIR != 0) {
+            if (r == 1) {
+              float n3 = u2f(mt.z);
+#pragma unroll
+              for (int i = 0; i < 8; ++i) n3 = min_raw(n3, hv[i] > prev ? hv[i] : FLT_MAX);
+              key3 = quad_min(n3);
+            }
+          }
         }
       }
       int32_t lab1 = 0, lab2 = 0;
@@ -529,10 +550,27 @@
       emit(act, mt.x, kind, lab1, lab2, (int32_t)(mt.y & 0xFFFFu));
       resid(act && kind == 0u, ws, xv);
       if constexpr (MARG) {
-        if (act && q == 0)
-          A.marg[mt.x] = (kind == 0u && gscale)
-                             ? s1g_base(s1g_margin(fminf(lbo, sRl[wave * S1_RING + slot]), ubw), sAd[lab1])
-                             : 0.0f;
+        float lb3 = 0.0f;
+        if constexpr (KM_S1_PAIR != 0) {
+          float xs = 0.0f;
+#pragma unroll
+          for (int u = 0; u < FQ / 4; ++u) {
+            xs = fmaf(xv[u].x, xv[u].x, xs);
+            xs = fmaf(xv[u].y, xv[u].y, xs);
+            xs = fmaf(xv[u].z, xv[u].z, xs);
+            xs = fmaf(xv[u].w, xv[u].w, xs);
+          }
+          const float xq = quad_sum(xs);
+          constexpr float RP = RHO * (1.0f + 2.0f * RHO);
+          lb3 = s1g_lb(key3, RP, s1g_row(s, fmaf(e1, s1g_xnorm(xq), e0), xq));
+        }
+        if (act && q == 0) {
+          const float lt = sRl[wave * S1_RING + slot];
+          const float mf = s1g_margin(fminf(lbo, lt), ubw);
+          const bool pr = KM_S1_PAIR != 0 && cnt == 2u && lab2 >= 0 && lbo < lb3 && !(mf > lthr);
+          const float bs = s1g_base(pr ? s1g_margin(lb3, ubw) : mf, sAd[lab1]);
+          A.marg[mt.x] = (kind == 0u && gscale) ? (pr ? s1g_pair_pack(bs, (uint32_t)lab2) : s1g_full(bs)) : 0.0f;
+        }
       }
     } else {
       (void)nb;
@@ -646,7 +684,7 @@
       lbT = s1g_lb(T, RP, gr);
       if (valid && !needy && q == 0)
         A.marg[row] =
-            (dec1 && gscale) ? s1g_base(s1g_margin(s1g_lb(h2, RP, gr), s1g_ub(m, RP, gr)), sAd[labm]) : 0.0f;
+            (dec1 && gscale) ? s1g_full(s1g_base(s1g_margin(s1g_lb(h2, RP, gr), s1g_ub(m, RP, gr)), sAd[labm])) : 0.0f;
     }
     if constexpr (BATCH) {
       emit(valid && !needy, row, dec1 ? 0u : 2u, labm, 0, old);
@@ -656,7 +694,9 @@
         const uint32_t nn = (uint32_t)__popcll(mrow);
         const uint32_t rk = (uint32_t)__popcll(mrow & ((1ull << c16) - 1ull));
         const uint32_t space = (uint32_t)S1_RING - rc;
-        const uint4 meta = make_uint4(row, (uint32_t)old | (cnt << 16), sm, f2u(la));
+        uint32_t mz = sm;
+        if constexpr (MARG && KM_S1_PAIR != 0) mz = f2u(quad_min(h2m));
+        const uint4 meta = make_uint4(row, (uint32_t)old | (cnt << 16), mz, f2u(la));
         auto stash = [&](uint32_t slot) {
           float4* xs = reinterpret_cast<float4*>(sRx + (wave * S1_RING + slot) * DP + FQ * q);
 #pragma unroll
@@ -969,7 +1009,9 @@
       acc[j] = s1g_acc_pass(acc[j], sv[j], j == atop ? top2 : top1, top1, reset != 0, &up, &dn);
       accud[j] = up;
       accud[k + j] = dn;
-    }
+      accud[2 * k + j] = s1g_up(sv[j] + (j == atop ? top2 : top1));
+    }
+    if (threadIdx.x == 0) accud[3 * k] = s1g_up(2.0f * s1g_up(top1 + top2));
   }
 }
 
@@ -985,7 +1027,15 @@
   int init;
   const int32_t* init_dev;
   const int* gate;
+  uint32_t* pair_cnt;
+  int pairs;
 };
+
+constexpr uint32_t S1_PAIR_OFF_BITS = 22u;
+static bool s1_pair_seg_ok(uint32_t seg) { return seg <= (1u << S1_PAIR_OFF_BITS); }
+__device__ __forceinline__ uint2 s1_pair_entry(uint32_t off, uint32_t label, float base) {
+  return make_uint2(off | (label << S1_PAIR_OFF_BITS), s1g_bits(base));
+}
 
 constexpr int S1G_UNITS = 2;
 constexpr uint32_t S1G_TRIP = 256u * S1G_UNITS;
@@ -1004,7 +1054,8 @@
   const uint64_t below = (1ull << lane) - 1ull;
   const bool init = A.init != 0 || (A.init_dev && *A.init_dev != 0);
   const uint32_t km1 = (uint32_t)(A.k - 1);
-  uint32_t cnt = 0;
+  const bool pairs = A.pairs != 0;
+  uint32_t cnt = 0, pcnt = 0;
   struct Trip {
     int4 lab[S1G_UNITS];
     float4 bs[S1G_UNITS];
@@ -1040,21 +1091,31 @@
       auto clampk = [&](int32_t v) -> uint32_t { return (uint32_t)v < km1 ? (uint32_t)v : km1; };
       const uint32_t l[4] = {clampk(T.lab[u].x), clampk(T.lab[u].y), clampk(T.lab[u].z), clampk(T.lab[u].w)};
       const float b[4] = {T.bs[u].x, T.bs[u].y, T.bs[u].z, T.bs[u].w};
-      bool ls[4];
-      uint32_t c = 0;
+      bool ls[4], lp[4];
+      uint32_t c = 0, cp = 0;
 #pragma unroll
       for (int i = 0; i < 4; ++i) {
-        ls[i] = row + i < r1 && (init || !s1g_keep(b[i], sUp[l[i]]));
+        const float up = sUp[l[i]];
+        const bool listed = row + i < r1 && (init || !s1g_keep(b[i], up));
+        lp[i] = listed && pairs && !init && s1g_pair_keep(b[i], up) && s1g_pair_partner(b[i]) <= km1;
+        ls[i] = listed && !lp[i];
         c += ls[i] ? 1u : 0u;
+        cp += lp[i] ? 1u : 0u;
       }
       const uint64_t b0 = __ballot((c & 1u) != 0u), b1 = __ballot((c & 2u) != 0u), b2 = __ballot((c & 4u) != 0u);
-      if ((b0 | b1 | b2) == 0ull) continue;
+      const uint64_t p0 = __ballot((cp & 1u) != 0u), p1 = __ballot((cp & 2u) != 0u), p2 = __ballot((cp & 4u) != 0u);
+      if ((b0 | b1 | b2 | p0 | p1 | p2) == 0ull) continue;
       uint32_t pos = cnt + (uint32_t)__popcll(b0 & below) + 2u * (uint32_t)__popcll(b1 & below) +
                      4u * (uint32_t)__popcll(b2 & below);
-#pragma unroll
-      for (int i = 0; i < 4; ++i)
+      uint32_t ppos = pcnt + (uint32_t)__popcll(p0 & below) + 2u * (uint32_t)__popcll(p1 & below) +
+                      4u * (uint32_t)__popcll(p2 & below);
+#pragma unroll
+      for (int i = 0; i < 4; ++i) {
         if (ls[i]) wl[pos++] = make_uint2((uint32_t)(row + i), l[i]);
+        if (lp[i]) wl[A.seg - 1u - ppos++] = s1_pair_entry((uint32_t)(row + i - r0), l[i], b[i]);
+      }
       cnt += (uint32_t)__popcll(b0) + 2u * (uint32_t)__popcll(b1) + 4u * (uint32_t)__popcll(b2);
+      pcnt += (uint32_t)__popcll(p0) + 2u * (uint32_t)__popcll(p1) + 4u * (uint32_t)__popcll(p2);
     }
   };
   const uint64_t rfull = r0 + (r1 - r0) / S1G_TRIP * S1G_TRIP;
@@ -1079,7 +1140,136 @@
     fetch_tail(base, tt);
     sift(base, tt);
   }
-  if (lane == 0) A.wl_cnt[gw] = cnt;
+  if (lane == 0) {
+    A.wl_cnt[gw] = cnt;
+    A.pair_cnt[gw] = pcnt;
+  }
+}
+
+#ifndef KM_S1_PAIR_LEAVE
+#define KM_S1_PAIR_LEAVE 2.0f
+#endif
+struct S1PairArgs {
+  const float* X;
+  const float* C32;
+  const float* cst;
+  int64_t n;
+  int k, d;
+  uint32_t seg;
+  const uint2* wl;
+  const uint32_t* pair_cnt;
+  const float* accud;
+  float* marg;
+  int32_t* labels;
+  QEntry* queue;
+  uint32_t* qcount;
+  uint2* chg;
+  uint32_t* chg_cnt;
+  const int* gate;
+};
+
+constexpr size_t s1_pair_lds(int dp, int k) { return (size_t)k * (dp + 4) * 4 + (size_t)3 * k * 4; }
+
+template <int NS2, int WAVES>
+__global__ __launch_bounds__(WAVES * 64) void k_s1_pair(S1PairArgs A) {
+  if (*A.gate) return;
+  constexpr int DP = 32 * NS2;
+  constexpr int FQ = 8 * NS2;
+  constexpr int CS = DP + 4;
+  extern __shared__ __attribute__((aligned(16))) char smem[];
+  float* sC = reinterpret_cast<float*>(smem);
+  float* sUp = sC + (size_t)A.k * CS;
+  float* sDn = sUp + A.k;
+  float* sSt = sDn + A.k;
+  for (int i = threadIdx.x; i < A.k * (DP / 4); i += WAVES * 64) {
+    const int j = i / (DP / 4), f = 4 * (i % (DP / 4));
+    float4 v = *reinterpret_cast<const float4*>(A.C32 + (size_t)j * DP + f);
+    v.x = f + 0 < A.d ? v.x : 0.0f;
+    v.y = f + 1 < A.d ? v.y : 0.0f;
+    v.z = f + 2 < A.d ? v.z : 0.0f;
+    v.w = f + 3 < A.d ? v.w : 0.0f;
+    *reinterpret_cast<float4*>(sC + j * CS + f) = v;
+  }
+  for (int i = threadIdx.x; i < 3 * A.k; i += WAVES * 64) sUp[i] = A.accud[i];
+  __syncthreads();
+
+  const int lane = threadIdx.x & 63, wave = threadIdx.x >> 6;
+  const int c16 = lane & 15, q = lane >> 4;
+  const float gam = A.cst[3];
+  const uint32_t n = (uint32_t)A.n;
+  const uint32_t km1 = (uint32_t)(A.k - 1);
+  const uint32_t gw = (uint32_t)__builtin_amdgcn_readfirstlane((int)(blockIdx.x * WAVES + wave));
+  const uint32_t np = (uint32_t)__builtin_amdgcn_readfirstlane((int)min(A.pair_cnt[gw], A.seg));
+  if (np == 0u) return;
+  const uint64_t r0 = (uint64_t)gw * A.seg;
+  const uint2* wlp = A.wl + (size_t)gw * A.seg;
+  QEntry* wq = A.queue + (size_t)gw * A.seg;
+  uint2* wc = A.chg + (size_t)gw * A.seg;
+  uint32_t qn = A.qcount[2 * gw], cc = A.chg_cnt[gw];
+  const uint64_t below = (1ull << lane) - 1ull;
+  constexpr uint32_t OFFM = (1u << S1_PAIR_OFF_BITS) - 1u;
+  auto efetch = [&](uint32_t g) { return wlp[A.seg - 1u - min(g * 64u + (uint32_t)lane, A.seg - 1u)]; };
+  auto pick = [&](uint32_t v, int i) {
+    return (uint32_t)__builtin_amdgcn_ds_bpermute((16 * i + c16) * 4, (int)v);
+  };
+  uint2 e = efetch(0u);
+  for (uint32_t g = 0u; g * 64u < np; ++g) {
+    const uint2 en = efetch(g + 1u);
+    float4 x[4][FQ / 4];
+    uint32_t row[4];
+#pragma unroll
+    for (int i = 0; i < 4; ++i) {
+      const uint32_t at = g * 64u + 16u * (uint32_t)i + (uint32_t)c16;
+      const uint64_t r = r0 + (pick(e.x, i) & OFFM);
+      row[i] = (at < np && r < n) ? (uint32_t)r : 0xFFFFFFFFu;
+      const float4* xr = reinterpret_cast<const float4*>(A.X + (size_t)min(row[i], n - 1u) * DP + FQ * q);
+#pragma unroll
+      for (int u = 0; u < FQ / 4; ++u) x[i][u] = xr[u];
+    }
+#pragma unroll
+    for (int i = 0; i < 4; ++i) {
+      if (g * 64u + 16u * (uint32_t)i >= np) break;
+      const bool act = row[i] != 0xFFFFFFFFu;
+      const float base = u2f(pick(e.y, i));
+      const uint32_t a = min(pick(e.x, i) >> S1_PAIR_OFF_BITS, km1), b = min(s1g_pair_partner(base), km1);
+      const float pa = s1_partial<FQ>(reinterpret_cast<const float4*>(sC + a * CS + FQ * q), x[i]);
+      const float pb = s1_partial<FQ>(reinterpret_cast<const float4*>(sC + b * CS + FQ * q), x[i]);
+      const float Da = quad_sum(pa), Db = quad_sum(pb);
+      S1_BOUNDS(Da, gam, Ua, La);
+      S1_BOUNDS(Db, gam, Ub, Lb);
+      const S1GPair r = s1g_pair_eval(s1g_pair_b3(base), sUp[a], a, b, La, Ua, Lb, Ub, sDn[a], sDn[b], sSt[a],
+                                      sSt[b], KM_S1_PAIR_LEAVE);
+      const bool one = act && q == 0;
+      if (one) A.marg[row[i]] = r.base;
+      const bool changed = one && r.decided && r.w != a;
+      const uint64_t mc = __ballot(changed);
+      if (mc) {
+        if (changed) {
+          A.labels[row[i]] = (int32_t)r.w;
+          wc[cc + (uint32_t)__popcll(mc & below)] = make_uint2(row[i], (a << 16) | r.w);
+        }
+        cc += (uint32_t)__popcll(mc);
+      }
+      const bool enq = one && !r.decided;
+      const uint64_t mq = __ballot(enq);
+      if (mq) {
+        if (enq) {
+          QEntry qe;
+          qe.row = row[i];
+          qe.i1 = r.w;
+          qe.i2 = r.o;
+          qe.kind = 1u;
+          wq[qn + (uint32_t)__popcll(mq & below)] = qe;
+        }
+        qn += (uint32_t)__popcll(mq);
+      }
+    }
+    e = en;
+  }
+  if (lane == 0) {
+    A.qcount[2 * gw] = qn;
+    A.chg_cnt[gw] = cc;
+  }
 }
 
 __global__ __launch_bounds__(256) void k_s1_apply(double* __restrict__ stats, double* __restrict__ full, int64_t len,
@@ -1367,11 +1557,37 @@
   hipError_t e = hipGetLastError();
   if (e != hipSuccess) return e;
   if (init == 2) return hipSuccess;
-  S1GateArgs a{labels, b.marg, g.n, g.k, seg, b.accud, b.wl, b.wl_cnt, init, init_dev, gate};
+  S1GateArgs a{labels, b.marg, g.n, g.k, seg, b.accud, b.wl, b.wl_cnt, init, init_dev, gate, b.pair_cnt,
+               (KM_S1_PAIR && s1_pair_seg_ok(seg)) ? 1 : 0};
   if (s1_geo_waves(g) == 12)
     hipLaunchKernelGGL(k_s1_gate<12>, dim3(nbk), dim3(12 * 64), 0, s, a);
   else
     hipLaunchKernelGGL(k_s1_gate<8>, dim3(nbk), dim3(8 * 64), 0, s, a);
+  return hipGetLastError();
+}
+
+hipError_t launch_s1_pair(const float* X, const float* C32, const float* cst, const Geometry& g, int32_t* labels,
+                          QEntry* queue, uint32_t* qcount, uint2* chg, uint32_t* chg_cnt, const S1GateBufs& b, int n_cu,
+                          const int* gate, hipStream_t s) {
+  if (g.n == 0) return hipSuccess;
+  if (!s1_gate_ok(g)) return hipErrorInvalidValue;
+  int nbk;
+  uint32_t seg;
+  (void)s1_grid(g, n_cu, &nbk, &seg);
+  if (!KM_S1_PAIR || !s1_pair_seg_ok(seg)) return hipSuccess;
+  const size_t lds = s1_pair_lds(g.dp, g.k);
+  if (lds > 160 * 1024) return hipErrorInvalidValue;
+  S1PairArgs a{X, C32, cst, g.n, g.k, g.d, seg, b.wl, b.pair_cnt, b.accud, b.marg, labels, queue, qcount, chg, chg_cnt,
+               gate};
+  const int w = s1_geo_waves(g);
+  if (g.dp == 64 && w == 12)
+    hipLaunchKernelGGL((k_s1_pair<2, 12>), dim3(nbk), dim3(12 * 64), lds, s, a);
+  else if (g.dp == 64 && w == 8)
+    hipLaunchKernelGGL((k_s1_pair<2, 8>), dim3(nbk), dim3(8 * 64), lds, s, a);
+  else if (g.dp == 32 && w == 8)
+    hipLaunchKernelGGL((k_s1_pair<1, 8>), dim3(nbk), dim3(8 * 64), lds, s, a);
+  else
+    return hipErrorInvalidValue;
   return hipGetLastError();
 }
 
diff --git a/assignment--2-group7-distributed-k-means_amd/engine.py b/assignment--2-group7-distributed-k-means_amd/engine.py
--- a/assignment--2-group7-distributed-k-means_amd/engine.py
+++ b/assignment--2-group7-distributed-k-means_amd/engine.py
@@ -295,6 +295,8 @@
         rows = ctypes.c_int64(-1)
         self._c(self.lib.km_gated_rows(self.ctx, ctypes.byref(rows)), "km_gated_rows")
         out["gated_rows"] = rows.value
+        self._c(self.lib.km_pair_rows(self.ctx, ctypes.byref(rows)), "km_pair_rows")
+        out["pair_rows"] = rows.value
         v = [ctypes.c_int32() for _ in range(5)]
         if self.lib.km_stats_route(self.ctx, *[ctypes.byref(x) for x in v]) == 0:
             for key, x in zip(("stats_route", "stats_cluster_ranges", "stats_kr", "stats_feature_ranges", "stats_fr"), v):
diff --git a/include/kmeans_amd.h b/include/kmeans_amd.h
--- a/include/kmeans_amd.h
+++ b/include/kmeans_amd.h
@@ -65,6 +65,7 @@
 int km_sync(km_ctx* ctx);
 int km_info_get(km_ctx* ctx, km_info* out);
 int km_gated_rows(km_ctx* ctx, int64_t* out);
+int km_pair_rows(km_ctx* ctx, int64_t* out);
 int km_stats_route(km_ctx* ctx, int32_t* route, int32_t* cluster_ranges, int32_t* kr, int32_t* feature_ranges,
                    int32_t* fr);
 
```
